# mmSir/SpatioTemporalEntropyModel

Hardware: AMD Instinct MI355X
Metric: frames/s (higher is better)
Workload: dtype f32; 1 GPU; configs[1]: SpatioTemporalPriorModel_Res(256,192) training step on mbt2018(192,192) latents, 16 septuplets x 7 frames x 256x256 per GPU, EMLoss, clip 1.0 + Adam 1e-4 / aux Adam 1e-3; per_gpu_batch=16, global_batch=16, parallelism=dp1, stream_priorities=latents=0,side=-1,compute=-1, stream_cu_masks=latents=block:160, plan_selectors=library defaults

## Files before the change

### __graft_entry__.py

```python
import os
import subprocess
import sys

REPO = os.path.dirname(os.path.abspath(__file__))
if REPO not in sys.path:
    sys.path.insert(0, REPO)


def build() -> None:
    env = dict(os.environ)
    jobs = str(min(8, os.cpu_count() or 1))
    subprocess.check_call(["make", "-C", os.path.join(REPO, "spatiotemporalentropymodel_amd", "csrc"), "-j", jobs], env=env)
    subprocess.check_call(["make", "-C", os.path.join(REPO, "oracle"), "all"], env=env)
    import spatiotemporalentropymodel_amd as pkg
    from spatiotemporalentropymodel_amd import _lib
    assert _lib.hip().stem_abi_version() == 5
    _lib.rans()
    _lib.frameio()
    _lib.roiio()


def smoke() -> None:
    from spatiotemporalentropymodel_amd.selfcheck import smoke_check
    smoke_check(verbose=True)


if __name__ == "__main__":
    build()
    if len(sys.argv) > 1 and sys.argv[1] == "smoke":
        smoke()
```

### spatiotemporalentropymodel_amd/_lib.py

```python
from __future__ import annotations

import ctypes as C
import os
import re

from . import _abi

_PKG = os.path.dirname(os.path.abspath(__file__))
HIP_SO = os.environ.get("STEM_HIP_LIBRARY") or os.path.join(_PKG, "libstem_hip.so")
RANS_SO = os.environ.get("STEM_RANS_LIBRARY") or os.path.join(_PKG, "libstem_rans.so")

FRAMEIO_SO = os.path.join(_PKG, "libstem_frameio.so")
ROIIO_SO = os.path.join(_PKG, "libstem_roiio.so")
DP_SO = os.environ.get("STEM_DP_LIBRARY") or os.path.join(_PKG, "libstem_dp.so")
_hip = None
_rans = None
_dp = None
_frameio = None
_roiio = None


class StemLibraryError(RuntimeError):
    pass


def _header(name):
    path = os.path.join(_PKG, "..", "include", name)
    if not os.path.exists(path):
        raise StemLibraryError(f"{path} is missing: the ctypes prototypes and structures are read from the C headers")
    return path


def _tables(header):
    protos = _abi.prototypes(_header(header))
    return protos, {n: args for n, (_, args) in protos.items()}, {n: res for n, (res, _) in protos.items() if res is not C.c_int}


_HIP_PROTO, _HIP_SIG, _RESTYPE = _tables("stem_hip.h")
_HIP_BATCH_PROTO, _HIP_BATCH_SIG, _ = _tables("stem_ar_batch.h")
_HIP_BLOCKS_PROTO, _HIP_BLOCKS_SIG, _ = _tables("stem_blocks.h")
_HIP_HYPERPRIOR_PROTO, _HIP_HYPERPRIOR_SIG, _ = _tables("stem_hyperprior.h")
_HIP_EBF_PROTO, _HIP_EBF_SIG, _ = _tables("stem_eb_filters.h")
_HIP_GDN1_PROTO, _HIP_GDN1_SIG, _ = _tables("stem_gdn1.h")
_HIP_VALIDATION_PROTO, _HIP_VALIDATION_SIG, _ = _tables("stem_validation.h")
_FRAMEIO_PROTO, _FRAMEIO_SIG, _ = _tables("stem_frameio.h")
_ROIIO_PROTO, _ROIIO_SIG, _ = _tables("stem_roiio.h")
_RANS_PROTO, _RANS_SIG, _RANS_RESTYPE = _tables("stem_rans.h")
_DP_PROTO, _DP_SIG, _ = _tables("stem_dp.h")
_STRUCTS = _abi.structs(_header("stem_hip.h"))


class PackDesc(C.Structure):
    _fields_ = _STRUCTS["stem_pack_desc"]


class F16PackDesc(C.Structure):
    _fields_ = _STRUCTS["stem_f16x2_pack_desc"]


class F16PairDesc(C.Structure):
    _fields_ = _STRUCTS["stem_f16x2_pair_desc"]


class UnpackDesc(C.Structure):
    _fields_ = _STRUCTS["stem_unpack_desc"]


class BiasFinalDesc(C.Structure):
    _fields_ = _STRUCTS["stem_bias_final_desc"]


class WaveSeg(C.Structure):
    _fields_ = _STRUCTS["stem_wave_seg"]


def _bind(lib, protos):
    for name, (restype, argtypes) in protos.items():
        fn = getattr(lib, name)
        fn.argtypes = argtypes
        fn.restype = restype
    return lib


def hip():
    global _hip
    if _hip is None:
        if not os.path.exists(HIP_SO):
            raise StemLibraryError(
                f"{HIP_SO} is missing: build it with `python -c 'import __graft_entry__ as g; g.build()'` "
                "(hipcc --offload-arch=gfx950).  There is no CPU fallback for the STEM kernels.")
        lib = C.CDLL(HIP_SO)
        for protos in (_HIP_PROTO, _HIP_BATCH_PROTO, _HIP_BLOCKS_PROTO, _HIP_HYPERPRIOR_PROTO, _HIP_EBF_PROTO, _HIP_GDN1_PROTO,
                       _HIP_VALIDATION_PROTO):
            _bind(lib, protos)
        _hip = lib
    return _hip


def frameio():
    global _frameio
    if _frameio is None:
        if not os.path.exists(FRAMEIO_SO):
            raise StemLibraryError(f"{FRAMEIO_SO} is missing: build it with `python -c 'import __graft_entry__ as g; g.build()'` "
                                   "(hipcc --offload-arch=gfx950).  There is no CPU fallback for the frame kernels.")
        _frameio = _bind(C.CDLL(FRAMEIO_SO), _FRAMEIO_PROTO)
    return _frameio


def check_frameio(rc: int):
    if rc != 0:
        raise RuntimeError((frameio().stem_frameio_last_error() or b"").decode() or f"libstem_frameio error {rc}")


def roiio():
    global _roiio
    if _roiio is None:
        if not os.path.exists(ROIIO_SO):
            raise StemLibraryError(f"{ROIIO_SO} is missing: build it with `python -c 'import __graft_entry__ as g; g.build()'` "
                                   "(hipcc --offload-arch=gfx950).  There is no CPU fallback for the frame kernels.")
        _roiio = _bind(C.CDLL(ROIIO_SO), _ROIIO_PROTO)
    return _roiio


def check_roiio(rc: int):
    if rc != 0:
        raise RuntimeError((roiio().stem_roiio_last_error() or b"").decode() or f"libstem_roiio error {rc}")


def rans():
    global _rans
    if _rans is None:
        if not os.path.exists(RANS_SO):
            raise StemLibraryError(f"{RANS_SO} is missing: run `make -C {os.path.join(_PKG, 'csrc')}`")
        _rans = _bind(C.CDLL(RANS_SO), _RANS_PROTO)
    return _rans


def check(rc: int):
    if rc != 0:
        raise RuntimeError((hip().stem_last_error() or b"").decode() or f"libstem_hip error {rc}")


def declared_hip_symbols():
    return sorted(_HIP_SIG)


def declared_hip_batch_symbols():
    return sorted(_HIP_BATCH_SIG)


def declared_hip_block_symbols():
    return sorted(_HIP_BLOCKS_SIG)


def declared_hip_hyperprior_symbols():
    return sorted(_HIP_HYPERPRIOR_SIG)


def declared_hip_eb_filters_symbols():
    return sorted(_HIP_EBF_SIG)


def declared_hip_gdn1_symbols():
    return sorted(_HIP_GDN1_SIG)


def declared_hip_validation_symbols():
    return sorted(_HIP_VALIDATION_SIG)


def declared_frameio_symbols():
    return sorted(_FRAMEIO_SIG)


def declared_roiio_symbols():
    return sorted(_ROIIO_SIG)


def header_macro(header, name):
    m = re.search(rf"^[ \t]*#[ \t]*define[ \t]+{name}[ \t]+(\d+)\b", open(_header(header)).read(), flags=re.M)
    if not m:
        raise StemLibraryError(f"include/{header} does not define {name} as an integer")
    return int(m.group(1))


def dp():
    global _dp
    if _dp is None:
        if not os.path.exists(DP_SO):
            raise StemLibraryError(f"{DP_SO} is missing: run `make -C {os.path.join(_PKG, 'csrc')}`")
        _dp = _bind(C.CDLL(DP_SO), _DP_PROTO)
    return _dp


def declared_dp_symbols():
    return sorted(_DP_SIG)


def declared_rans_symbols():
    return sorted(_RANS_SIG)
```

### spatiotemporalentropymodel_amd/config.py

```python
from __future__ import annotations

import contextlib
import dataclasses
import os
from dataclasses import dataclass


@dataclass
class StemRuntimeConfig:
    analysis_f16x3: bool = True
    first_layer_f16x3: bool = True
    engine_f16x3: bool = True
    engine_strided_f16x3: bool = True
    engine_transposed_f16x3: bool = True
    engine_ctx_f16x3: bool = True
    engine_wgrad_f16x3: bool = True
    engine_records: bool = True
    layers_f16x3: bool = True
    layers_f16x3_maxpix: int = 1 << 30
    layers_wide_minpix: int = 32768
    trainer_overwrite_grads: bool = True
    adam_block_max: bool = True
    engine_overlap: bool = True
    engine_split_pack: bool = True
    engine_pack_pair: bool = True
    engine_branch: bool = True
    stream_prio: str = ""
    stream_cumask: str = ""
    dp_threaded: int = 3
    dp_min_bytes: int = 8 << 20
    dist_backend: str = ""
    dist_single: bool = False
    pin_ranks: bool = True
    ar_persistent: bool = True
    ar_stepwise: bool = False
    ar_force_batch: bool = False
    ar_concurrent: bool = True
    ar_no_batch: bool = False


_ENV = {
    "analysis_f16x3": "STEM_F16X3", "first_layer_f16x3": "STEM_C4GDN_F16X3", "engine_f16x3": "STEM_ENGINE_F16X3",
    "engine_strided_f16x3": "STEM_ENGINE_STRIDED_F16X3", "engine_transposed_f16x3": "STEM_ENGINE_TRANSPOSED_F16X3", "engine_ctx_f16x3": "STEM_ENGINE_CTX_F16X3",
    "engine_wgrad_f16x3": "STEM_ENGINE_WGRAD_F16X3", "engine_records": "STEM_ENGINE_RECORDS", "layers_f16x3": "STEM_LAYERS_F16X3",
    "layers_f16x3_maxpix": "STEM_LAYERS_F16X3_MAXPIX", "layers_wide_minpix": "STEM_LAYERS_WIDE_MINPIX",
    "adam_block_max": "STEM_ADAM_BLOCK_MAX", "trainer_overwrite_grads": "STEM_TRAINER_OVERWRITE_GRADS", "engine_overlap": "STEM_ENGINE_OVERLAP",
    "engine_split_pack": "STEM_ENGINE_SPLIT_PACK", "engine_pack_pair": "STEM_ENGINE_PACK_PAIR", "engine_branch": "STEM_ENGINE_BRANCH",
    "stream_prio": "STEM_STREAM_PRIO", "stream_cumask": "STEM_STREAM_CUMASK", "dp_min_bytes": "STEM_DP_MIN_BYTES", "dp_threaded": "STEM_DP_THREADED",
    "dist_backend": "STEM_DIST_BACKEND", "dist_single": "STEM_DIST_SINGLE", "pin_ranks": "STEM_PIN_RANKS",
    "ar_persistent": "STEM_AR_PERSISTENT", "ar_stepwise": "STEM_AR_STEPWISE",
    "ar_force_batch": "STEM_AR_FORCE_BATCH", "ar_concurrent": "STEM_AR_CONCURRENT", "ar_no_batch": "STEM_AR_NO_BATCH",
}


def _parse(kind, text):
    if kind is bool:
        return text.strip() not in ("", "0", "false", "False", "no", "off")
    if kind is int:
        return int(text)
    return text


def from_env(environ=None) -> StemRuntimeConfig:
    environ = os.environ if environ is None else environ
    cfg = StemRuntimeConfig()
    for f in dataclasses.fields(cfg):
        name = _ENV[f.name]
        if name in environ:
            setattr(cfg, f.name, _parse(type(f.default), environ[name]))
    return cfg


_RUNTIME = None
_SNAPSHOT = None
_OVERRIDES = {}


def _snapshot():
    env = os.environ
    return tuple(env.get(v) for v in _ENV.values())


def runtime() -> StemRuntimeConfig:
    global _RUNTIME, _SNAPSHOT
    snap = _snapshot()
    if _RUNTIME is None or snap != _SNAPSHOT:
        _RUNTIME, _SNAPSHOT = from_env(), snap
        for k, v in _OVERRIDES.items():
            setattr(_RUNTIME, k, v)
    return _RUNTIME


def reload() -> StemRuntimeConfig:
    global _RUNTIME
    _RUNTIME = None
    return runtime()


@contextlib.contextmanager
def override(**fields):
    cfg = runtime()
    unknown = [k for k in fields if not hasattr(cfg, k)]
    if unknown:
        raise AttributeError(f"StemRuntimeConfig has no field(s) {unknown}")
    old = {k: (_OVERRIDES[k] if k in _OVERRIDES else None, k in _OVERRIDES, getattr(cfg, k)) for k in fields}
    try:
        for k, v in fields.items():
            _OVERRIDES[k] = v
            setattr(runtime(), k, v)
        yield runtime()
    finally:
        for k, (ov, had, val) in old.items():
            if had:
                _OVERRIDES[k] = ov
            else:
                _OVERRIDES.pop(k, None)
            setattr(runtime(), k, ov if had else val)
```

### spatiotemporalentropymodel_amd/csrc/optim.hip

```cpp
#include "stem_common.h"

namespace {

__global__ __launch_bounds__(256) void sumsq_kernel(const f32x4 *g4, const float *g, size_t n4, size_t n, double *part)
{
    __shared__ double red[256];
    double s = 0.0;
    for (size_t i = (size_t)blockIdx.x * 256 + threadIdx.x; i < n4; i += (size_t)gridDim.x * 256) {
        const f32x4 v = g4[i];
        s += (double)v[0] * v[0] + (double)v[1] * v[1] + (double)v[2] * v[2] + (double)v[3] * v[3];
    }
    if (blockIdx.x == 0)
        for (size_t i = n4 * 4 + threadIdx.x; i < n; i += 256) s += (double)g[i] * g[i];
    red[threadIdx.x] = s;
    __syncthreads();
    for (int k = 128; k > 0; k >>= 1) {
        if (threadIdx.x < k) red[threadIdx.x] += red[threadIdx.x + k];
        __syncthreads();
    }
    if (threadIdx.x == 0) part[blockIdx.x] = red[0];
}
__global__ __launch_bounds__(256) void sumsq_final_kernel(const double *part, int nparts, double *acc, int overwrite)
{
    __shared__ double red[256];
    double s = 0.0;
    for (int i = threadIdx.x; i < nparts; i += 256) s += part[i];
    red[threadIdx.x] = s;
    __syncthreads();
    for (int k = 128; k > 0; k >>= 1) {
        if (threadIdx.x < k) red[threadIdx.x] += red[threadIdx.x + k];
        __syncthreads();
    }
    if (threadIdx.x == 0) acc[0] = overwrite ? red[0] : acc[0] + red[0];
}

__global__ __launch_bounds__(256) void adam_kernel(float *p, float *g, float *m, float *v, size_t n, const double *sumsq,
                                                   float max_norm, float gscale, float step_size, float b1, float b2,
                                                   float inv_sqrt_bc2, float eps, const float *dev_scal, int zero_g)
{
    if (dev_scal) {
        step_size = dev_scal[0];
        inv_sqrt_bc2 = dev_scal[1];
    }
    float coef = gscale;
    if (max_norm > 0.f && sumsq) {
        const float total = (float)sqrt(sumsq[0]) * gscale;
        coef *= fminf(max_norm / (total + 1e-6f), 1.0f);
    }
    for (size_t i = (size_t)blockIdx.x * 256 + threadIdx.x; i < n; i += (size_t)gridDim.x * 256) {
        const float gi = g[i] * coef;
        if (zero_g) g[i] = 0.f;
        const float mi = m[i] + (gi - m[i]) * (1.f - b1);
        const float vi = v[i] * b2 + (1.f - b2) * gi * gi;
        m[i] = mi;
        v[i] = vi;
        p[i] -= step_size * (mi / (sqrtf(vi) * inv_sqrt_bc2 + eps));
    }
}

__global__ __launch_bounds__(256) void adam_bmax_kernel(float *p, float *g, float *m, float *v, size_t n, const double *sumsq,
                                                        float max_norm, float gscale, float step_size, float b1, float b2,
                                                        float inv_sqrt_bc2, float eps, int zero_g, float *bmax)
{
    float coef = gscale;
    if (max_norm > 0.f && sumsq) {
        const float total = (float)sqrt(sumsq[0]) * gscale;
        coef *= fminf(max_norm / (total + 1e-6f), 1.0f);
    }
    const size_t base = (size_t)blockIdx.x * STEM_ADAM_CHUNK;
    float mx = 0.f;
#pragma unroll 1
    for (int k0 = 0; k0 < STEM_ADAM_CHUNK / 256; k0 += 4) {
        float gi[4], mi[4], vi[4], pi[4];
        size_t idx[4];
#pragma unroll
        for (int u = 0; u < 4; ++u) {
            idx[u] = base + (size_t)(k0 + u) * 256 + threadIdx.x;
            const bool ok = idx[u] < n;
            const size_t j = ok ? idx[u] : 0;
            gi[u] = ok ? g[j] : 0.f;
            mi[u] = ok ? m[j] : 0.f;
            vi[u] = ok ? v[j] : 0.f;
            pi[u] = ok ? p[j] : 0.f;
        }
#pragma unroll
        for (int u = 0; u < 4; ++u) {
            if (idx[u] >= n) continue;
            const float gs = gi[u] * coef;
            if (zero_g) g[idx[u]] = 0.f;
            const float mn = mi[u] + (gs - mi[u]) * (1.f - b1);
            const float vn = vi[u] * b2 + (1.f - b2) * gs * gs;
            m[idx[u]] = mn;
            v[idx[u]] = vn;
            const float pn = pi[u] - step_size * (mn / (sqrtf(vn) * inv_sqrt_bc2 + eps));
            p[idx[u]] = pn;
            mx = fmaxf(mx, fabsf(pn));
        }
    }
    mx = wave_max(mx);
    if ((threadIdx.x & 63) == 0) bmax[blockIdx.x * 4 + (threadIdx.x >> 6)] = mx;
}

__global__ void adam_prepare_kernel(long long *step, const float *lr, float b1, float b2, float *scal)
{
    const long long t = step[0] + 1;
    step[0] = t;
    const double bc1 = 1.0 - pow((double)b1, (double)t), bc2 = 1.0 - pow((double)b2, (double)t);
    scal[0] = (float)((double)lr[0] / bc1);
    scal[1] = (float)(1.0 / sqrt(bc2));
}

__global__ void counter_add_kernel(long long *ctr, long long inc) { ctr[0] += inc; }

__global__ __launch_bounds__(256) void clip_scale_kernel(float *g, size_t n, const double *sumsq, float max_norm)
{
    const float coef = fminf(max_norm / ((float)sqrt(sumsq[0]) + 1e-6f), 1.0f);
    if (coef >= 1.0f) return;
    for (size_t i = (size_t)blockIdx.x * 256 + threadIdx.x; i < n; i += (size_t)gridDim.x * 256) g[i] *= coef;
}

__global__ __launch_bounds__(256) void axpy_kernel(float *y, const float *x, float a, size_t n)
{
    for (size_t i = (size_t)blockIdx.x * 256 + threadIdx.x; i < n; i += (size_t)gridDim.x * 256) y[i] += a * x[i];
}

}

namespace {
int sumsq_impl(const float *g, size_t n, double *acc, int overwrite, void *stream);
}
STEM_EXPORT int stem_sumsq(const float *g, size_t n, double *acc, void *stream) { return sumsq_impl(g, n, acc, 0, stream); }
STEM_EXPORT int stem_sumsq_set(const float *g, size_t n, double *acc, void *stream) { return sumsq_impl(g, n, acc, 1, stream); }
namespace {
int sumsq_impl(const float *g, size_t n, double *acc, int overwrite, void *stream)
{
    STEM_CHECK_ARG(g && acc, "stem_sumsq: null pointer");
    if (n == 0) {
        if (overwrite && hipMemsetAsync(acc, 0, sizeof(double), (hipStream_t)stream) != hipSuccess) return -2;
        return 0;
    }
    const bool al = (((uintptr_t)g) & 15) == 0;
    const size_t n4 = al ? n / 4 : 0;
    size_t nb = cdivz(n4 ? n4 : 1, 256);
    if (nb > STEM_SUMSQ_SCRATCH) nb = STEM_SUMSQ_SCRATCH;
    hipLaunchKernelGGL(sumsq_kernel, dim3((unsigned)nb), dim3(256), 0, (hipStream_t)stream,
                       reinterpret_cast<const f32x4 *>(g), g, n4, n, acc + 1);
    hipLaunchKernelGGL(sumsq_final_kernel, dim3(1), dim3(256), 0, (hipStream_t)stream, acc + 1, (int)nb, acc, overwrite);
    STEM_LAUNCH_CHECK("sumsq");
    return 0;
}
}

STEM_EXPORT int stem_adam_step(float *p, const float *g, float *m, float *v, size_t n, const double *sumsq, float max_norm,
                               float gscale, float lr, float beta1, float beta2, float eps, int step, void *stream)
{
    STEM_CHECK_ARG(p && g && m && v && step >= 1, "stem_adam_step: bad arguments");
    if (n == 0) return 0;
    const double bc1 = 1.0 - pow((double)beta1, step), bc2 = 1.0 - pow((double)beta2, step);
    size_t nb = cdivz(n, 256);
    if (nb > 4096) nb = 4096;
    hipLaunchKernelGGL(adam_kernel, dim3((unsigned)nb), dim3(256), 0, (hipStream_t)stream, p, const_cast<float *>(g), m, v, n, sumsq, max_norm,
                       gscale, (float)(lr / bc1), beta1, beta2, (float)(1.0 / sqrt(bc2)), eps, (const float *)nullptr, 0);
    STEM_LAUNCH_CHECK("adam");
    return 0;
}

STEM_EXPORT int stem_adam_step_zero(float *p, float *g, float *m, float *v, size_t n, const double *sumsq, float max_norm,
                                    float gscale, float lr, float beta1, float beta2, float eps, int step, void *stream)
{
    STEM_CHECK_ARG(p && g && m && v && step >= 1, "stem_adam_step_zero: bad arguments");
    if (n == 0) return 0;
    const double bc1 = 1.0 - pow((double)beta1, step), bc2 = 1.0 - pow((double)beta2, step);
    size_t nb = cdivz(n, 256);
    if (nb > 4096) nb = 4096;
    hipLaunchKernelGGL(adam_kernel, dim3((unsigned)nb), dim3(256), 0, (hipStream_t)stream, p, g, m, v, n, sumsq, max_norm,
                       gscale, (float)(lr / bc1), beta1, beta2, (float)(1.0 / sqrt(bc2)), eps, (const float *)nullptr, 1);
    STEM_LAUNCH_CHECK("adam_zero");
    return 0;
}

STEM_EXPORT size_t stem_adam_chunk(void) { return STEM_ADAM_CHUNK; }

STEM_EXPORT int stem_adam_step_bmax(float *p, float *g, float *m, float *v, size_t n, const double *sumsq, float max_norm,
                                    float gscale, float lr, float beta1, float beta2, float eps, int step, int zero_grad, float *bmax,
                                    void *stream)
{
    STEM_CHECK_ARG(p && g && m && v && bmax && step >= 1, "stem_adam_step_bmax: bad arguments");
    if (n == 0) return 0;
    const double bc1 = 1.0 - pow((double)beta1, step), bc2 = 1.0 - pow((double)beta2, step);
    hipLaunchKernelGGL(adam_bmax_kernel, dim3((unsigned)cdivz(n, STEM_ADAM_CHUNK)), dim3(256), 0, (hipStream_t)stream, p, g, m, v, n, sumsq,
                       max_norm, gscale, (float)(lr / bc1), beta1, beta2, (float)(1.0 / sqrt(bc2)), eps, zero_grad, bmax);
    STEM_LAUNCH_CHECK("adam_bmax");
    return 0;
}

STEM_EXPORT int stem_adam_step_dev(float *p, const float *g, float *m, float *v, size_t n, const double *sumsq, float max_norm,
                                   float gscale, const float *lr_dev, float beta1, float beta2, float eps, long long *step_dev,
                                   float *scal_dev, void *stream)
{
    STEM_CHECK_ARG(p && g && m && v && lr_dev && step_dev && scal_dev, "stem_adam_step_dev: null pointer");
    if (n == 0) return 0;
    hipLaunchKernelGGL(adam_prepare_kernel, dim3(1), dim3(1), 0, (hipStream_t)stream, step_dev, lr_dev, beta1, beta2, scal_dev);
    size_t nb = cdivz(n, 256);
    if (nb > 4096) nb = 4096;
    hipLaunchKernelGGL(adam_kernel, dim3((unsigned)nb), dim3(256), 0, (hipStream_t)stream, p, const_cast<float *>(g), m, v, n, sumsq, max_norm,
                       gscale, 0.f, beta1, beta2, 0.f, eps, (const float *)scal_dev, 0);
    STEM_LAUNCH_CHECK("adam_dev");
    return 0;
}

STEM_EXPORT int stem_counter_add(long long *ctr, long long inc, void *stream)
{
    STEM_CHECK_ARG(ctr, "stem_counter_add: null pointer");
    hipLaunchKernelGGL(counter_add_kernel, dim3(1), dim3(1), 0, (hipStream_t)stream, ctr, inc);
    STEM_LAUNCH_CHECK("counter_add");
    return 0;
}

STEM_EXPORT int stem_clip_scale(float *g, size_t n, const double *sumsq, float max_norm, void *stream)
{
    STEM_CHECK_ARG(g && sumsq && max_norm > 0.f, "stem_clip_scale: bad arguments");
    if (n == 0) return 0;
    size_t nb = cdivz(n, 256);
    if (nb > 4096) nb = 4096;
    hipLaunchKernelGGL(clip_scale_kernel, dim3((unsigned)nb), dim3(256), 0, (hipStream_t)stream, g, n, sumsq, max_norm);
    STEM_LAUNCH_CHECK("clip_scale");
    return 0;
}

STEM_EXPORT int stem_axpy(float *y, const float *x, float a, size_t n, void *stream)
{
    STEM_CHECK_ARG(y && x, "stem_axpy: null pointer");
    if (n == 0) return 0;
    size_t nb = cdivz(n, 256);
    if (nb > 4096) nb = 4096;
    hipLaunchKernelGGL(axpy_kernel, dim3((unsigned)nb), dim3(256), 0, (hipStream_t)stream, y, x, a, n);
    STEM_LAUNCH_CHECK("axpy");
    return 0;
}
```

### spatiotemporalentropymodel_amd/csrc/tape.hip

```cpp
#include <algorithm>
#include <array>
#include <type_traits>
#include <utility>
#include <vector>

#include "stem_common.h"

namespace {

constexpr int TAPE_MAXI = 40, TAPE_MAXF = 6;
enum { TAPE_CALL = 0, TAPE_WAIT = 1, TAPE_EVENT_RECORD = 2, TAPE_EVENT_WAIT = 3 };

struct TapeEntry {
    int kind;
    void *fn;
    int ni, nf;
    long long iv[TAPE_MAXI];
    long long idelta[TAPE_MAXI];
    double fv[TAPE_MAXF];
    hipStream_t s0, s1;
    hipEvent_t ev;
    bool dynamic;
};

struct Tape {
    std::vector<TapeEntry> e;
    std::vector<hipEvent_t> owned;
};

template <size_t... I, size_t... Fx>
int call_seq(void *fn, const long long *iv, const double *fv, std::index_sequence<I...>, std::index_sequence<Fx...>)
{
    using Fn = int (*)(decltype((void)I, 0LL)..., decltype((void)Fx, 0.0)...);
    return reinterpret_cast<Fn>(fn)(iv[I]..., fv[Fx]...);
}
template <size_t NI>
int call_ni(void *fn, const long long *iv, int nf, const double *fv)
{
    switch (nf) {
    case 0: return call_seq(fn, iv, fv, std::make_index_sequence<NI>{}, std::make_index_sequence<0>{});
    case 1: return call_seq(fn, iv, fv, std::make_index_sequence<NI>{}, std::make_index_sequence<1>{});
    case 2: return call_seq(fn, iv, fv, std::make_index_sequence<NI>{}, std::make_index_sequence<2>{});
    case 3: return call_seq(fn, iv, fv, std::make_index_sequence<NI>{}, std::make_index_sequence<3>{});
    case 4: return call_seq(fn, iv, fv, std::make_index_sequence<NI>{}, std::make_index_sequence<4>{});
    case 5: return call_seq(fn, iv, fv, std::make_index_sequence<NI>{}, std::make_index_sequence<5>{});
    default: return call_seq(fn, iv, fv, std::make_index_sequence<NI>{}, std::make_index_sequence<6>{});
    }
}
using Caller = int (*)(void *, const long long *, int, const double *);
template <size_t... N>
constexpr auto make_callers(std::index_sequence<N...>) -> std::array<Caller, sizeof...(N)>
{
    return {{&call_ni<N>...}};
}
const auto kCallers = make_callers(std::make_index_sequence<TAPE_MAXI + 1>{});

static_assert(TAPE_MAXF <= 8, "SSE arguments beyond xmm7 go to the stack and would interleave with the integer overflow area");
template <class T>
constexpr bool tape_int_class = (std::is_integral<T>::value || std::is_enum<T>::value || std::is_pointer<T>::value) && sizeof(T) <= 8;
template <class T>
constexpr bool tape_sse_class = std::is_same<T, float>::value || std::is_same<T, double>::value;
template <class... A>
constexpr bool tape_recordable(int (*)(A...))
{
    constexpr int ni = (0 + ... + (tape_int_class<A> ? 1 : 0)), nf = (0 + ... + (tape_sse_class<A> ? 1 : 0));
    return ni + nf == (int)sizeof...(A) && ni <= TAPE_MAXI && nf <= TAPE_MAXF;
}
#define STEM_TAPE_ENTRY(name) \
    static_assert(tape_recordable(&name), #name ": prototype outside the launch tape's calling contract (csrc/tape.hip)");
#include "tape_entries.inc"
#undef STEM_TAPE_ENTRY

#define STEM_TAPE_ENTRY(name) reinterpret_cast<const void *>(&name),
const void *const kRecordable[] = {
#include "tape_entries.inc"
};
#undef STEM_TAPE_ENTRY

}

STEM_EXPORT int stem_tape_entry_recordable(void *fn)
{
    return std::find(std::begin(kRecordable), std::end(kRecordable), (const void *)fn) != std::end(kRecordable) ? 1 : 0;
}

STEM_EXPORT void *stem_tape_create(void) { return new Tape(); }

STEM_EXPORT void stem_tape_destroy(void *tape)
{
    Tape *t = static_cast<Tape *>(tape);
    if (!t) return;
    for (hipEvent_t ev : t->owned) (void)hipEventDestroy(ev);
    delete t;
}

STEM_EXPORT int stem_tape_length(void *tape) { return tape ? (int)static_cast<Tape *>(tape)->e.size() : -1; }

STEM_EXPORT int stem_tape_add_call(void *tape, void *fn, int nargs, const unsigned char *kinds, const long long *ivals, const double *fvals,
                                   const long long *ideltas)
{
    Tape *t = static_cast<Tape *>(tape);
    STEM_CHECK_ARG(t && fn && nargs >= 0 && (nargs == 0 || (kinds && ivals && fvals)), "stem_tape_add_call: null argument");
    TapeEntry en;
    memset(&en, 0, sizeof(en));
    en.kind = TAPE_CALL;
    en.fn = fn;
    for (int i = 0; i < nargs; ++i) {
        if (kinds[i] != 0) {
            STEM_CHECK_ARG(en.nf < TAPE_MAXF, "stem_tape_add_call: more than %d float arguments", TAPE_MAXF);
            en.fv[en.nf++] = fvals[i];
        } else {
            STEM_CHECK_ARG(en.ni < TAPE_MAXI, "stem_tape_add_call: more than %d integer-class arguments", TAPE_MAXI);
            en.iv[en.ni] = ivals[i];
            en.idelta[en.ni] = ideltas ? ideltas[i] : 0;
            en.dynamic = en.dynamic || en.idelta[en.ni] != 0;
            ++en.ni;
        }
    }
    t->e.push_back(en);
    return (int)t->e.size() - 1;
}

STEM_EXPORT int stem_tape_add_wait(void *tape, void *waiting, void *signalling)
{
    Tape *t = static_cast<Tape *>(tape);
    STEM_CHECK_ARG(t, "stem_tape_add_wait: null tape");
    TapeEntry en;
    memset(&en, 0, sizeof(en));
    en.kind = TAPE_WAIT;
    en.s0 = (hipStream_t)waiting;
    en.s1 = (hipStream_t)signalling;
    if (hipEventCreateWithFlags(&en.ev, hipEventDisableTiming) != hipSuccess) {
        stem_set_error("stem_tape_add_wait: hipEventCreate failed");
        return -2;
    }
    t->owned.push_back(en.ev);
    t->e.push_back(en);
    return (int)t->e.size() - 1;
}

STEM_EXPORT int stem_tape_add_event(void *tape, void *event, void *stream, int wait)
{
    Tape *t = static_cast<Tape *>(tape);
    STEM_CHECK_ARG(t && event, "stem_tape_add_event: null argument");
    TapeEntry en;
    memset(&en, 0, sizeof(en));
    en.kind = wait ? TAPE_EVENT_WAIT : TAPE_EVENT_RECORD;
    en.s0 = (hipStream_t)stream;
    en.ev = (hipEvent_t)event;
    t->e.push_back(en);
    return (int)t->e.size() - 1;
}

STEM_EXPORT int stem_tape_replay(void *tape, int lo, int hi, long long n)
{
    Tape *t = static_cast<Tape *>(tape);
    STEM_CHECK_ARG(t && lo >= 0 && hi <= (int)t->e.size() && lo <= hi, "stem_tape_replay: bad range [%d, %d)", lo, hi);
    for (int i = lo; i < hi; ++i) {
        const TapeEntry &en = t->e[i];
        switch (en.kind) {
        case TAPE_CALL: {
            int rc;
            if (en.dynamic) {
                long long iv[TAPE_MAXI];
                for (int k = 0; k < en.ni; ++k) iv[k] = en.iv[k] + n * en.idelta[k];
                rc = kCallers[en.ni](en.fn, iv, en.nf, en.fv);
            } else {
                rc = kCallers[en.ni](en.fn, en.iv, en.nf, en.fv);
            }
            if (rc != 0) return -(i + 1);
            break;
        }
        case TAPE_WAIT:
            if (hipEventRecord(en.ev, en.s1) != hipSuccess || hipStreamWaitEvent(en.s0, en.ev, 0) != hipSuccess) {
                stem_set_error("stem_tape_replay: stream hand-over of entry %d failed", i);
                return -(i + 1);
            }
            break;
        case TAPE_EVENT_RECORD:
            if (hipEventRecord(en.ev, en.s0) != hipSuccess) {
                stem_set_error("stem_tape_replay: event record of entry %d failed", i);
                return -(i + 1);
            }
            break;
        default:
            if (hipStreamWaitEvent(en.s0, en.ev, 0) != hipSuccess) {
                stem_set_error("stem_tape_replay: event wait of entry %d failed", i);
                return -(i + 1);
            }
        }
    }
    return 0;
}

STEM_EXPORT int stem_tape_set_iarg(void *tape, int entry, int arg, long long value)
{
    Tape *t = static_cast<Tape *>(tape);
    STEM_CHECK_ARG(t && entry >= 0 && entry < (int)t->e.size() && t->e[entry].kind == TAPE_CALL && arg >= 0 && arg < t->e[entry].ni,
                   "stem_tape_set_iarg: no integer argument %d in entry %d", arg, entry);
    t->e[entry].iv[arg] = value;
    return 0;
}

STEM_EXPORT int stem_tape_set_farg(void *tape, int entry, int arg, double pattern)
{
    Tape *t = static_cast<Tape *>(tape);
    STEM_CHECK_ARG(t && entry >= 0 && entry < (int)t->e.size() && t->e[entry].kind == TAPE_CALL && arg >= 0 && arg < t->e[entry].nf,
                   "stem_tape_set_farg: no float argument %d in entry %d", arg, entry);
    t->e[entry].fv[arg] = pattern;
    return 0;
}

STEM_EXPORT int stem_zero_bytes(void *dst, size_t nbytes, void *stream)
{
    STEM_CHECK_ARG(dst || !nbytes, "stem_zero_bytes: null pointer");
    if (nbytes && hipMemsetAsync(dst, 0, nbytes, (hipStream_t)stream) != hipSuccess) {
        stem_set_error("stem_zero_bytes: hipMemsetAsync failed");
        return -2;
    }
    return 0;
}

STEM_EXPORT int stem_stream_flag_create(void **flag)
{
    STEM_CHECK_ARG(flag, "stem_stream_flag_create: null pointer");
    int dev = 0, ok = 0;
    if (hipGetDevice(&dev) != hipSuccess || hipDeviceGetAttribute(&ok, hipDeviceAttributeCanUseStreamWaitValue, dev) != hipSuccess || !ok) {
        stem_set_error("stem_stream_flag_create: this device / runtime has no stream wait-value operation");
        return -3;
    }
    void *p = nullptr;
    if (hipExtMallocWithFlags(&p, 8, hipMallocSignalMemory) != hipSuccess || !p) {
        stem_set_error("stem_stream_flag_create: hipExtMallocWithFlags(hipMallocSignalMemory) failed");
        return -2;
    }
    *static_cast<volatile uint64_t *>(p) = 0;
    *flag = p;
    return 0;
}

STEM_EXPORT int stem_stream_flag_destroy(void *flag)
{
    if (flag && hipFree(flag) != hipSuccess) {
        stem_set_error("stem_stream_flag_destroy: hipFree failed");
        return -2;
    }
    return 0;
}

STEM_EXPORT int stem_stream_flag_wait_ge(void *flag, unsigned value, void *stream)
{
    STEM_CHECK_ARG(flag, "stem_stream_flag_wait_ge: null flag");
    if (hipStreamWaitValue32((hipStream_t)stream, flag, value, hipStreamWaitValueGte, 0xffffffffu) != hipSuccess) {
        stem_set_error("stem_stream_flag_wait_ge: hipStreamWaitValue32 failed");
        return -2;
    }
    return 0;
}

STEM_EXPORT int stem_stream_flag_write(void *flag, unsigned value, void *stream)
{
    STEM_CHECK_ARG(flag, "stem_stream_flag_write: null flag");
    if (stream == (void *)-1) {
        __atomic_store_n(static_cast<uint32_t *>(flag), value, __ATOMIC_RELEASE);
        return 0;
    }
    if (hipStreamWriteValue32((hipStream_t)stream, flag, value, 0) != hipSuccess) {
        stem_set_error("stem_stream_flag_write: hipStreamWriteValue32 failed");
        return -2;
    }
    return 0;
}

STEM_EXPORT int stem_copy_d2d(void *dst, const void *src, size_t nbytes, void *stream)
{
    STEM_CHECK_ARG(dst && src, "stem_copy_d2d: null pointer");
    if (nbytes && hipMemcpyAsync(dst, src, nbytes, hipMemcpyDeviceToDevice, (hipStream_t)stream) != hipSuccess) {
        stem_set_error("stem_copy_d2d: hipMemcpyAsync failed");
        return -2;
    }
    return 0;
}
```

### spatiotemporalentropymodel_amd/engine.py

```python
from __future__ import annotations

import collections

import torch

from . import _lib
from . import config as _config
from . import functional as F
from . import layers as _layers

class _Switch:

    def __init__(self, field):
        self.field = field

    def __get__(self, obj, owner=None):
        return getattr(_config._RUNTIME or _config.runtime(), self.field)


class _Act:
    __slots__ = ("x", "p", "rec")

    def __init__(self, x, p=None, rec=None):
        self.x, self.p, self.rec = x, p, rec

    def planes(self, record=True):
        if self.p is None:
            self.p = F.F16Planes.split(self.x, src_q=self.rec.data_ptr() if record and self.rec is not None else None)
        return self.p

    def channels(self, c0, c1):
        return _Act(self.x[:, c0:c1], None if self.p is None else self.p.channels(c0, c1))


_Face = collections.namedtuple("_Face", "kind N C flip taps")


class _Layer:

    def __init__(self, mod, kind, eng):
        self.mod, self.kind, self.eng = mod, kind, eng
        self.R = mod.kernel_size
        self.stride, self.pad = mod.stride, mod.padding
        self.opad = getattr(mod, "output_padding", 0)
        self.K, self.C = mod.out_channels, mod.in_channels
        self.masked = getattr(mod, "_masked", 0)
        self.wp_fwd = self.wp_dgrad = None
        self.need_dgrad = True
        self.fx3 = False
        self.wg3 = False
        self.taps = 0
        self.fx3s = False
        self.fx3t = False
        self.wp6_fwd = self.wp6_dgrad = None
        self._slabs = {}
        self.pending = None
        self.lane = 0

    def fx3_eligible(self):
        return self.kind == "conv" and not self.masked and _layers.f16x3_same_shape(self.stride, self.R, self.pad, self.C, self.K)

    def fx3_masked_eligible(self):
        return (self.kind == "conv" and bool(self.masked) and not self.need_dgrad
                and _layers.f16x3_same_shape(self.stride, self.R, self.pad, self.C, self.K, k_multiple=4))

    def fx3s_eligible(self):
        n_out, n_red = (self.K, self.C) if self.kind == "conv" else (self.C, self.K)
        return (self.stride == 2 and not self.masked and n_red % 32 == 0 and n_out % 4 == 0 and self.R * self.R <= 25
                and (self.kind == "conv" or self.need_dgrad))

    def fx3t_eligible(self):
        return (self.fx3s and self.R % 2 == 1 and self.R >= 3 and self.pad == self.R // 2 and self.C % 32 == 0 and self.K % 32 == 0
                and (self.kind == "conv" or self.opad == 1))

    def wg3_eligible(self):
        return self.kind == "conv" and _layers.f16x3_same_shape(self.stride, self.R, self.pad, self.C, self.K)

    def set_faces(self):
        K, C, conv = self.K, self.C, self.kind == "conv"
        fwd = dgrad = _Face("f32", K, C, 0, 0)
        if self.fx3:
            fwd, dgrad = _Face("gen", K, C, 0, self.taps), _Face("gen", C, K, 1, 0)
        elif self.fx3s:
            if conv:
                fwd, dgrad = _Face("gen", K, C, 0, 0), (_Face("phases", C, K, 2, 0) if self.fx3t else dgrad)
            else:
                fwd, dgrad = (_Face("phases", K, C, 2, 0) if self.fx3t else fwd), _Face("gen", C, K, 0, 0)
        self.faces = (fwd, dgrad if self.need_dgrad else None)

    def alloc_packs(self, device):
        bufs = []
        for face in self.faces:
            if face is None:
                bufs += [None, None]
            elif face.kind == "f32":
                bufs += [torch.empty(self.K * self.C * self.R * self.R, device=device, dtype=torch.float32), None]
            else:
                bufs += [None, torch.zeros(F.f16x2_gen_weight_bytes(face.N, face.C, self.R, self.R), device=device, dtype=torch.uint8)]
        self.wp_fwd, self.wp6_fwd, self.wp_dgrad, self.wp6_dgrad = bufs
        if self.fx3s and self.wp_fwd is None:
            self.wp_fwd = torch.empty(0, device=device)

    def role_descs(self, role):
        face = self.faces[role]
        if face is None:
            return [], []
        if face.kind == "f32":
            return [self._desc32(role)], []
        wp = self.wp6_dgrad if role else self.wp6_fwd
        return [], [_lib.F16PackDesc(self.mod.weight.data_ptr(), wp.data_ptr(), face.N, face.C, self.R, self.R, face.flip, face.taps)]

    def pair_desc(self):
        a, b = self.role_descs(0), self.role_descs(1)
        if a[0] or b[0] or not a[1]:
            return None
        w = self.mod.weight
        A, Bd = int(w.shape[0]), int(w.shape[1])
        roles = []
        for d in (a[1][0], b[1][0] if b[1] else None):
            if d is None:
                roles += [None, 0, 0]
                continue
            rows_b = int(d.flip != 0)
            assert (d.N, d.C) == ((Bd, A) if rows_b else (A, Bd)), "pair pack: a role image must be a transpose of the tensor itself"
            roles += [d.wp, rows_b | (int(d.flip) << 1), int(d.taps)]
        return _lib.F16PairDesc(w.data_ptr(), A, Bd, self.R, self.R, roles[0], roles[1], roles[2], roles[3], roles[4], roles[5], None, 0, 0)

    def _desc32(self, role):
        w = self.mod.weight
        conv = self.kind == "conv"
        if role == 0:
            return _lib.PackDesc(w.data_ptr(), self.wp_fwd.data_ptr(), self.K, self.C, self.R, self.R,
                                 F.PACK_CONV_FWD if conv else F.PACK_DECONV_FWD, self.masked)
        return _lib.PackDesc(w.data_ptr(), self.wp_dgrad.data_ptr(), self.K, self.C, self.R, self.R,
                             F.PACK_CONV_DGRAD if conv else F.PACK_DECONV_DGRAD, (1 | (self.masked & 4)) if self.masked else 0)

    def forward(self, a, act=F.ACT_NONE, out=None, planes=False):
        self.eng.ensure_packed()
        face, m = self.faces[0], self.mod
        epi = F.GEN_EPI_LRELU if act == F.ACT_LRELU else F.GEN_EPI_BIAS
        if face.kind == "gen":
            return _Act(*F.conv2d_f16x3_gen(a.planes(), self.wp6_fwd, m.bias, self.K, self.R, self.R, self.stride, self.pad,
                                            epi=epi, out=out, want_planes=planes, taps=self.taps))
        if face.kind == "phases":
            return _Act(*F.tconv2d_f16x3(a.planes(), self.wp6_fwd, m.bias, self.K, self.R, epi=epi, out=out, want_planes=planes))
        self.eng._wait_fwd32_packs()
        if self.kind == "conv":
            if self.masked and not self.masked & 4:
                act |= F.CONV_MASKED_A
            return _Act(F.conv2d_fwd(a.x, self.wp_fwd, m.bias, self.K, self.R, self.R, self.stride, self.pad, act, out=out))
        return _Act(F.deconv2d_fwd(a.x, self.wp_fwd, m.bias, self.K, self.R, self.R, self.stride, self.pad, self.opad, act, out=out))

    def fwd(self, x, act=F.ACT_NONE, out=None):
        return self.forward(_Act(x), act, out=out).x

    def input_grad(self, dy, xact=None, planes=False, x_shape=None):
        face = self.faces[1]
        epi = F.GEN_EPI_DACT if xact is not None else F.GEN_EPI_BIAS
        if face.kind == "gen":
            return _Act(*F.conv2d_f16x3_gen(dy.planes(), self.wp6_dgrad, None, self.C, self.R, self.R, self.stride, self.pad,
                                            epi=epi, z=xact, want_planes=planes))
        if face.kind == "phases":
            return _Act(*F.tconv2d_f16x3(dy.planes(), self.wp6_dgrad, None, self.C, self.R, epi=epi, z=xact, want_planes=planes,
                                         fine_hw=tuple(xact.shape[2:]) if xact is not None else None))
        x_shape = xact.shape if xact is not None else x_shape
        if self.kind == "conv":
            return _Act(F.conv2d_dgrad(dy.x, self.wp_dgrad, x_shape, self.K, self.R, self.R, self.stride, self.pad, xact=xact))
        return _Act(F.deconv2d_dgrad(dy.x, self.wp_dgrad, x_shape, self.K, self.R, self.R, self.stride, self.pad, self.opad, xact=xact))

    def reads_dy_planes(self, x):
        return self.faces[1].kind != "f32" if self.faces[1] is not None else (self.wg3 and x.p is not None)

    def weight_grad(self, x, dy):
        at_hand = (x.p is not None) + (dy.p is not None)
        if self.fx3t:
            fn, args = self._wgrad_t, ((x.planes(), dy.planes()) if self.kind == "conv" else (dy.planes(), x.planes())) + (dy.x,)
        elif self.wg3 and at_hand >= (2 if self.need_dgrad else 1):
            fn, args = self._wgrad3, (x.planes(record=False), dy.planes(record=False), dy.x)
        else:
            fn, args = self._wgrad, (x.x, dy.x)
        side = self.eng.side_stream(dy.x.device, self.lane)
        if side is None:
            return fn(*args)
        F.stream_wait(side, F.cur_stream(dy.x.device))
        with F.on_stream(side):
            fn(*args)
        for t in args:
            (t.data if isinstance(t, F.F16Planes) else t).record_stream(side)

    def _wgrad_t(self, fine_p, coarse_p, dy):
        conv = self.kind == "conv"
        Kk = self.K if conv else self.C
        key = ("fp16t",) + tuple(fine_p.shape)
        if key not in self._slabs:
            splits, elems = F.wgrad_f16x3_strided_plan(fine_p.shape, Kk, self.R, self.R, self.stride, self.pad)
            self._slabs[key] = (torch.empty(elems, device=dy.device, dtype=torch.float32), splits,
                                torch.empty(splits * Kk, device=dy.device, dtype=torch.float32))
        dwp, splits, bpart = self._slabs[key]
        gb = _grad_of(self.mod.bias) if self.mod.bias is not None else None
        F.conv2d_wgrad_f16x3_strided(fine_p, coarse_p, Kk, self.R, self.R, self.stride, self.pad, dwp, splits,
                                     bias_part=bpart if (conv and gb is not None) else None)
        self.pending_bias = None
        if gb is not None and conv:
            self.pending_bias = _lib.BiasFinalDesc(bpart.data_ptr(), gb.data_ptr(), self.K, splits, int(self.eng.accumulate_grads), 0)
        elif gb is not None:
            F.bias_grad(dy, gb, accumulate=self.eng.accumulate_grads)
        self.pending = (dwp, splits)

    def _wgrad3(self, xp, dyp, dy):
        key = ("fp16",) + tuple(xp.shape)
        if key not in self._slabs:
            splits, elems = F.wgrad_f16x3_plan(xp.shape, self.K, self.R, self.R, self.pad)
            self._slabs[key] = (torch.empty(elems, device=dy.device, dtype=torch.float32), splits,
                                torch.empty(splits * self.K, device=dy.device, dtype=torch.float32))
        dwp, splits, bpart = self._slabs[key]
        gb = _grad_of(self.mod.bias) if self.mod.bias is not None else None
        self.pending_bias = F.conv2d_wgrad_f16x3(xp, dyp, self.K, self.R, self.R, self.pad, dwp, splits, db=gb, bias_part=bpart,
                                                 accumulate_db=self.eng.accumulate_grads, defer_bias=True)
        self.pending = (dwp, splits)

    def _wgrad(self, x, dy):
        m = self.mod
        gb = _grad_of(m.bias)
        deconv = self.kind == "deconv"
        key = tuple(x.shape)
        key = key + (F.nhwc_ld(x), F.nhwc_ld(dy))
        fresh = key not in self._slabs
        if fresh:
            splits, elems = F.wgrad_plan(x.shape, self.K, self.R, self.R, self.stride, self.pad, deconv=deconv)
            self._slabs[key] = (torch.empty(elems, device=x.device, dtype=torch.float32), splits)
        dwp, splits = self._slabs[key]
        defer = gb is not None
        if deconv:
            _, b = F.deconv2d_wgrad(x, dy, self.K, self.R, self.R, self.stride, self.pad, self.opad, db_out=gb, dwp=dwp, unpack=False,
                                    table_valid=not fresh, accumulate_db=self.eng.accumulate_grads, defer_bias=defer)
        else:
            _, b = F.conv2d_wgrad(x, dy, self.K, self.R, self.R, self.stride, self.pad, db_out=gb, dwp=dwp, unpack=False,
                                  table_valid=not fresh, accumulate_db=self.eng.accumulate_grads, defer_bias=defer)
        self.pending_bias = b if defer else None
        self.pending = (dwp, splits)

    def unpack_desc(self):
        dwp, splits = self.pending
        self.pending = None
        return _lib.UnpackDesc(dwp.data_ptr(), _grad_of(self.mod.weight).data_ptr(), self.K, self.C, self.R, self.R, splits,
                               (F.UNPACK_DECONV if self.kind == "deconv" else 0) | (F.UNPACK_ACCUMULATE if self.eng.accumulate_grads else 0))


def _attach_block_maxima(d, numel, maxima, flat, ch=None):
    off = (d.w - flat.data_ptr()) // 4
    if (d.w - flat.data_ptr()) % 4 or off < 0 or off + numel > flat.numel():
        return False
    ch = ch or F.adam_chunk()
    d.bmax, d.b0 = maxima.data_ptr(), off // ch
    d.nb = (off + numel - 1) // ch - d.b0 + 1
    return True


def _grad_of(p):
    if p.grad is None:
        owner = getattr(p, "_flat_grad_view", None)
        p.grad = owner if owner is not None else torch.zeros_like(p, memory_format=torch.contiguous_format)
    return p.grad


class StemEngine:
    def __init__(self, model, has_tpm: bool, has_spm: bool, residual: bool):
        _config.runtime()
        self.m = model
        eb_filters = tuple(model.entropy_bottleneck.filters)
        if eb_filters != (3, 3, 3, 3):
            raise ValueError(f"StemEngine: the fused schedule is built for an EntropyBottleneck with filters=(3, 3, 3, 3), this model's "
                             f"has filters={eb_filters}; its module-by-module forward (model(y_cur, y_conditioned)) and autograd work")
        self.has_tpm, self.has_spm, self.residual = has_tpm, has_spm, residual
        L = lambda mod: _Layer(mod, "conv", self)
        D = lambda mod: _Layer(mod, "deconv", self)
        self.HE = [L(model.HE[0]), L(model.HE[2]), L(model.HE[4])]
        self.HD = [D(model.HD[0]), D(model.HD[2]), L(model.HD[4])]
        self.TPM = [L(model.TPM[0]), L(model.TPM[2]), L(model.TPM[4])] if has_tpm else None
        self.CTX = L(model.context_prediction) if has_spm else None
        self.EPM = [L(model.EPM[0]), L(model.EPM[2]), L(model.EPM[4])]
        self.nprior = 1 + int(has_tpm) + int(has_spm)
        self.layers = self.HE + self.HD + (self.TPM or []) + ([self.CTX] if has_spm else []) + self.EPM
        for first in [self.HE[0]] + ([self.TPM[0]] if has_tpm else []) + ([self.CTX] if has_spm else []):
            first.need_dgrad = False
        self._pack_key = None
        self._side = {}
        self._checked = False
        self._dgrad_pack_event = None
        self._fwd32_pack_event = None
        self.accumulate_grads = True
        self._events = {}
        self._select_fx3()

    def _select_fx3(self):
        for l in self.layers:
            l.fx3 = self.use_fx3 and l.fx3_eligible()
            l.taps = 0
            l.fx3s = False
        if self.use_fx3 and self.use_fx3s:
            if self.HE[0].fx3 and self.HE[1].fx3s_eligible():
                self.HE[1].fx3s = True
                self.HE[2].fx3s = self.HE[2].fx3s_eligible() and self.HE[1].K % 32 == 0
            if self.HD[2].fx3 and self.HD[1].fx3s_eligible():
                self.HD[1].fx3s = True
                self.HD[0].fx3s = self.HD[0].fx3s_eligible() and self.HD[1].C % 32 == 0
        if self.use_fx3t and self.use_wg3:
            for l in self.HE[1:] + self.HD[:2]:
                l.fx3t = l.fx3t_eligible()
            if not (self.HE[1].fx3t and self.HE[2].fx3t and self.HE[0].fx3):
                self.HE[1].fx3t = self.HE[2].fx3t = False
            if not (self.HD[0].fx3t and self.HD[1].fx3t and self.HD[2].fx3):
                self.HD[0].fx3t = self.HD[1].fx3t = False
        if self.has_spm and self.use_fx3 and self.use_ctx3 and self.CTX.fx3_masked_eligible():
            self.CTX.fx3 = True
            self.CTX.taps = F.masked_live_taps(self.CTX.R, self.CTX.R, "B" if self.CTX.masked & 4 else "A")
        P = self.HE[0].C
        for group, need_aligned in ((self.TPM, False), (self.EPM, True)):
            if group and not (all(l.fx3 for l in group) and (not need_aligned or P % 32 == 0)):
                for l in group:
                    l.fx3 = False
        for l in self.layers:
            l.wg3 = self.use_fx3 and self.use_wg3 and l.wg3_eligible()
            l.set_faces()

    use_fx3 = _Switch("engine_f16x3")
    use_records = _Switch("engine_records")
    use_fx3s = _Switch("engine_strided_f16x3")
    use_fx3t = _Switch("engine_transposed_f16x3")
    use_ctx3 = _Switch("engine_ctx_f16x3")
    use_wg3 = _Switch("engine_wgrad_f16x3")

    overlap_wgrad = _Switch("engine_overlap")

    split_pack = _Switch("engine_split_pack")

    def side_stream(self, device, lane=0):
        if not self.overlap_wgrad or device.type != "cuda" or lane < 0:
            return None
        st = self._side.get(lane)
        if st is None or st.device != device:
            st = self._side[lane] = F.make_stream(device, "side")
        return st

    branch_streams = _Switch("engine_branch")

    def _branch(self, device, which=0):
        if not self.branch_streams or device.type != "cuda":
            return None
        bs = getattr(self, "_bstreams", None)
        if bs is None:
            bs = self._bstreams = {}
        st = bs.get(which)
        if st is None or st.device != device:
            st = bs[which] = F.make_stream(device, "branch")
        return st

    def ensure_packed(self, block_max=None, split=True):
        if self._checked:
            return
        if self._weights_key() == self._pack_key:
            return
        have = [l.wp_fwd if l.faces[0].kind == "f32" else l.wp6_fwd for l in self.layers]
        if any(h is None or h.device != l.mod.weight.device for h, l in zip(have, self.layers)):
            for l in self.layers:
                l.alloc_packs(l.mod.weight.device)
        dev = self.layers[0].mod.weight.device
        if block_max is not None and self.pack_pair and self._pack_pairs(*block_max):
            self._pack_key = self._weights_key()
            return
        side = self.side_stream(dev) if split and self.split_pack and not torch.cuda.is_current_stream_capturing() else None
        if not split:
            for st in list(self._side.values()) + list(getattr(self, "_bstreams", {}).values()):
                F.stream_wait(F.cur_stream(dev), st)
            self._dgrad_pack_event = None
        roles = ((0, 1), (1, 2)) if side is not None else ((0, 2),)
        for lo, hi in roles:
            on_side = side is not None and lo == 1
            if on_side:
                F.stream_wait(side, F.cur_stream(dev))
            with F.on_stream(side if on_side else None):
                both = [l.role_descs(r) for l in self.layers for r in range(lo, hi)]
                descs = [d for a, _ in both for d in a]
                descs6 = [d for _, b in both for d in b]
                if descs6 and block_max is not None:
                    ch = F.adam_chunk()
                    for d in descs6:
                        _attach_block_maxima(d, d.N * d.C * d.R * d.S, *block_max, ch)
                if descs6:
                    F.pack_weights_f16x2_multi((_lib.F16PackDesc * len(descs6))(*descs6))
                bs = self._branch(dev) if (descs and side is not None and not on_side and lo == 0 and hi == 1) else None
                if descs and bs is not None:
                    F.stream_wait(bs, F.cur_stream(dev))
                    with F.on_stream(bs):
                        F.pack_weights_multi((_lib.PackDesc * len(descs))(*descs))
                        self._fwd32_pack_event = self._events.setdefault("fwd32", torch.cuda.Event())
                        F.event_record(self._fwd32_pack_event, bs)
                elif descs:
                    F.pack_weights_multi((_lib.PackDesc * len(descs))(*descs))
                    if not on_side:
                        self._fwd32_pack_event = None
                if on_side:
                    self._dgrad_pack_event = self._events.setdefault("dgrad", torch.cuda.Event())
                    F.event_record(self._dgrad_pack_event, side)
        self._pack_key = self._weights_key()

    def _weights_key(self):
        return tuple((_layers.weight_epoch(l.mod.weight), l.mod.weight._version, l.mod.weight.data_ptr()) for l in self.layers)

    pack_pair = _Switch("engine_pack_pair")

    def _pack_pairs(self, maxima, flat):
        descs = [l.pair_desc() for l in self.layers]
        if any(d is None for d in descs):
            return False
        ch = F.adam_chunk()
        if not all(_attach_block_maxima(d, d.A * d.B * d.R * d.S, maxima, flat, ch) for d in descs):
            return False
        F.pack_weights_f16x2_pair_multi((_lib.F16PairDesc * len(descs))(*descs))
        self._dgrad_pack_event = None
        return True

    def unpack_all(self):
        for lane in sorted({l.lane for l in self.layers}):
            self._group_ready([l for l in self.layers if l.lane == lane], [])

    grad_ready_hook = None

    def _group_ready(self, layers, extra_params):
        dev = layers[0].mod.weight.device
        side = self.side_stream(dev, layers[0].lane)
        if side is None:
            return self._group_ready_on_stream(layers, extra_params)
        F.stream_wait(side, F.cur_stream(dev))
        with F.on_stream(side):
            self._group_ready_on_stream(layers, extra_params)

    def _group_ready_on_stream(self, layers, extra_params):
        bdescs = [l.pending_bias for l in layers if getattr(l, "pending_bias", None) is not None]
        for l in layers:
            l.pending_bias = None
        if bdescs:
            F.bias_grad_final_multi(bdescs)
        descs = [l.unpack_desc() for l in layers if l.pending is not None]
        if descs:
            arr = (_lib.UnpackDesc * len(descs))(*descs)
            F.unpack_wgrads_multi(arr)
        if self.grad_ready_hook is not None:
            params = [p for l in layers for p in (l.mod.weight, l.mod.bias) if p is not None] + list(extra_params)
            if params:
                hook = self.grad_ready_hook
                F.tape_py(lambda: hook(params))

    def join_side_stream(self):
        for st in self._side.values():
            F.stream_wait(F.cur_stream(st.device), st)

    def _wait_fwd32_packs(self):
        if self._fwd32_pack_event is not None:
            F.event_wait(F.cur_stream(), self._fwd32_pack_event)

    def _wait_dgrad_packs(self):
        if self._dgrad_pack_event is not None:
            F.event_wait(F.cur_stream(), self._dgrad_pack_event)
            self._dgrad_pack_event = None

    def forward(self, y_cur, y_cond, training: bool, rate_coef=None):
        self.ensure_packed()
        self._checked = True
        try:
            return self._forward(y_cur, y_cond, training, rate_coef)
        finally:
            self._checked = False

    @staticmethod
    def _chain_forward(layers, a, out=None, planes=True):
        acts = [a]
        for i, l in enumerate(layers):
            nxt = layers[i + 1] if i + 1 < len(layers) else None
            acts.append(l.forward(acts[-1], F.ACT_LRELU if nxt else F.ACT_NONE, out=None if nxt else out,
                                  planes=planes and nxt is not None and nxt.faces[0].kind != "f32"))
        return acts

    @staticmethod
    def _chain_backward(layers, xs, dy, planes=False):
        for i in range(len(layers) - 1, -1, -1):
            l = layers[i]
            if l.faces[1] is not None and l.faces[1].kind != "f32":
                dy.planes()
            l.weight_grad(xs[i], dy)
            if l.faces[1] is None:
                return None
            dy = l.input_grad(dy, xact=xs[i].x if i else None, x_shape=xs[i].x.shape,
                              planes=layers[i - 1].reads_dy_planes(xs[i - 1]) if i else planes)
        return dy

    def _forward(self, y_cur, y_cond, training: bool, rate_coef=None):
        m = self.m
        yc, yd = F.to_nhwc(y_cur.detach()), F.to_nhwc(y_cond.detach())
        B, Cin, H, W = yc.shape
        dev = yc.device
        eb, gc = m.entropy_bottleneck, m.gaussian_conditional
        fused = rate_coef is not None
        assert not fused or training, "the fused glue is the TRAINING forward"
        k = {}
        target = t_hat = y_hat = None
        ep = training or self.has_spm
        rec = {}
        if fused:
            slot = gc._noise_slot(yc) if self.has_spm else {}
            he_in, target, t_hat, y_hat = F.prior_prologue(yc, yd, self.residual, True, self.has_spm, records=rec if self.use_fx3 and self.use_records else None, **slot)
        else:
            he_in = F.empty_nhwc(B, 2 * Cin, H, W, dev)
            F.copy_channels(yc, he_in[:, :Cin])
            F.copy_channels(yd, he_in[:, Cin:])
        P = 2 * Cin
        epm_in = F.empty_nhwc(B, self.nprior * P, H, W, dev)
        o_tp, o_hp = (0, P) if self.has_tpm else (None, 0)
        o_ctx = o_hp + P
        bs = self._branch(dev)
        main = F.cur_stream(dev) if bs is not None else None
        if bs is not None:
            F.stream_wait(bs, main)
        acts = k["acts"] = {}
        acts["he_in"] = _Act(he_in, rec=rec.get("in"))
        acts["yd"] = _Act(yd, rec=rec.get("in"))
        ctx_split_done = None
        if self.has_spm and fused:
            acts["t_hat"] = _Act(t_hat, rec=rec.get("t_hat"))
            if self.CTX.fx3 and rec.get("t_hat") is not None and self.side_stream(dev) is not None:
                side = self.side_stream(dev)
                F.stream_wait(side, F.cur_stream(dev))
                with F.on_stream(side):
                    acts["t_hat"].planes()
                    ctx_split_done = self._events.setdefault("ctx_split", torch.cuda.Event())
                    F.event_record(ctx_split_done, side)
                t_hat.record_stream(side)

        if fused and self.HE[0].fx3 and self.has_tpm and self.TPM[0].fx3 and Cin % 32 == 0 and rec.get("in") is not None:
            acts["yd"] = _Act(yd, acts["he_in"].planes().channels(Cin, 2 * Cin))
            if bs is not None:
                F.stream_wait(bs, main)

        tp0 = tp2 = None
        if self.has_tpm:
            _, acts["tp0"], acts["tp2"], _ = self._chain_forward(self.TPM, acts["yd"], out=epm_in[:, o_tp:o_tp + P], planes=ep)
            tp0, tp2 = acts["tp0"].x, acts["tp2"].x
        with F.on_stream(bs):
            _, acts["he0"], acts["he2"], z = self._chain_forward(self.HE, acts["he_in"], planes=ep)
            z = z.x
            pack = F.eb_pack(eb._tensors14())
            if fused:
                if self.HD[0].fx3t and self.use_records:
                    z_hat, lik_z, k["dlik_z"], part_z, rec["z_hat"] = F.eb_forward_train(z, pack, rate_coef[0], bound=eb._lik_bound, record=True,
                                                                                         **eb._noise_slot(z))
                else:
                    z_hat, lik_z, k["dlik_z"], part_z = F.eb_forward_train(z, pack, rate_coef[0], bound=eb._lik_bound, **eb._noise_slot(z))
            elif training:
                z_hat, lik_z = F.eb_forward(z, pack, noise=eb._noise_like(z))
            else:
                z_hat, lik_z = F.eb_forward(z, pack, medians=eb._medians_vec())
            acts["z_hat"], acts["hd0"], acts["hd2"], _ = self._chain_forward(self.HD, _Act(z_hat, rec=rec.get("z_hat")), out=epm_in[:, o_hp:o_hp + P], planes=ep)
        if not fused:
            target = F.sub(yc, yd) if self.residual else (yc if F.nhwc_ld(yc) == Cin else F.copy_channels(yc, F.empty_nhwc(B, Cin, H, W, dev)))
        if self.has_spm:
            if not fused:
                t_hat = F.add(target, gc._noise_like(target)) if training else F.round_(target)
                acts["t_hat"] = _Act(t_hat)
            if ctx_split_done is not None:
                F.event_wait(F.cur_stream(dev), ctx_split_done)
            self.CTX.forward(acts["t_hat"], out=epm_in[:, o_ctx:o_ctx + P])
        if bs is not None:
            F.stream_wait(main, bs)
        acts["epm_in"], acts["e0"], acts["e2"], gp = self._chain_forward(self.EPM, _Act(epm_in), planes=ep)
        gp = gp.x
        scales, means = gp[:, :Cin], gp[:, Cin:]
        if fused:
            dgp = F.empty_nhwc(B, 2 * Cin, H, W, dev)
            gc_out, lik_y, k["dlik_y"], part_y, k["qg"] = F.gc_forward_train(
                target, scales, means, rate_coef[0], scale_bound=gc._scale_bound, lik_bound=gc._lik_bound,
                backward=(dgp[:, :Cin], dgp[:, Cin:]), record=self.EPM[0].fx3 and self.use_records, **gc._noise_slot(target))
            k["dgp"] = dgp
            k["loss3"] = F.em_loss_finalize(part_y, part_z, rate_coef[1])
            if not self.has_spm:
                y_hat = gc_out
        else:
            noise = gc._noise_like(target) if training else None
            gc_out, lik_y = F.gc_forward(target, scales, means, noise=noise, scale_bound=gc._scale_bound, lik_bound=gc._lik_bound)
            if self.has_spm:
                y_hat = F.add(t_hat, yd if F.nhwc_ld(yd) == Cin else F.copy_channels(yd, F.empty_nhwc(B, Cin, H, W, dev))) if self.residual else t_hat
            else:
                y_hat = gc_out
        k.update(he_in=he_in, he0=acts["he0"].x, he2=acts["he2"].x, z_hat=z_hat, pack=pack, hd0=acts["hd0"].x, hd2=acts["hd2"].x,
                 epm_in=epm_in, tp0=tp0, tp2=tp2, yd=yd, t_hat=t_hat, e0=acts["e0"].x, e2=acts["e2"].x, gp=gp, gc_out=gc_out,
                 offs=(o_tp, o_hp, o_ctx), P=P, Cin=Cin)
        return y_hat, lik_y, lik_z, k

    def eval_rate(self, y_cur, y_cond, num_pixels, acc=None, weight=1.0):
        self.ensure_packed()
        self._checked = True
        try:
            return self._eval_rate(y_cur, y_cond, num_pixels, acc, weight)
        finally:
            self._checked = False

    def _eval_rate(self, y_cur, y_cond, num_pixels, acc, weight):
        m = self.m
        yc, yd = F.to_nhwc(y_cur.detach()), F.to_nhwc(y_cond.detach())
        B, Cin, H, W = yc.shape
        dev = yc.device
        eb, gc = m.entropy_bottleneck, m.gaussian_conditional
        ep = self.has_spm
        he_in, target, t_hat, y_hat = F.prior_prologue(yc, yd, self.residual, False, self.has_spm, records=None)
        P = 2 * Cin
        epm_in = F.empty_nhwc(B, self.nprior * P, H, W, dev)
        o_tp, o_hp = (0, P) if self.has_tpm else (None, 0)
        o_ctx = o_hp + P
        bs = self._branch(dev)
        main = F.cur_stream(dev) if bs is not None else None
        if bs is not None:
            F.stream_wait(bs, main)
        if self.has_tpm:
            self._chain_forward(self.TPM, _Act(yd), out=epm_in[:, o_tp:o_tp + P], planes=ep)
        with F.on_stream(bs):
            z = self._chain_forward(self.HE, _Act(he_in), planes=ep)[-1].x
            z_hat, lik_z, part_z = F.eb_forward_eval_rate(z, F.eb_pack(eb._tensors14()), eb._medians_vec())
            self._chain_forward(self.HD, _Act(z_hat), out=epm_in[:, o_hp:o_hp + P], planes=ep)
        if self.has_spm:
            self.CTX.forward(_Act(t_hat), out=epm_in[:, o_ctx:o_ctx + P])
        if bs is not None:
            F.stream_wait(main, bs)
            for t in (lik_z, part_z):
                t.record_stream(main)
        gp = self._chain_forward(self.EPM, _Act(epm_in), planes=ep)[-1].x
        gc_out, lik_y, part_y = F.gc_forward_eval_rate(target, gp[:, :Cin], gp[:, Cin:], scale_bound=gc._scale_bound, lik_bound=gc._lik_bound)
        if acc is None:
            acc = torch.zeros(4, dtype=torch.float64, device=dev)
        loss3 = F.em_loss_accumulate(part_y, part_z, -1.0 / num_pixels, acc, weight=weight)
        return (y_hat if self.has_spm else gc_out), lik_y, lik_z, loss3

    def backward(self, k, dlik_y, dlik_z):
        m = self.m
        gc = m.gaussian_conditional
        Cin, P = k["Cin"], k["P"]
        o_tp, o_hp, o_ctx = k["offs"]
        gp, acts = k["gp"], k["acts"]
        B, _, H, W = gp.shape
        self._wait_dgrad_packs()
        if k.get("dgp") is not None and dlik_y is k.get("dlik_y"):
            dgp, qg = k["dgp"], k["qg"]
        else:
            dgp = F.empty_nhwc(B, 2 * Cin, H, W, gp.device)
            qg = F.gc_backward(k["gc_out"], gp[:, :Cin], gp[:, Cin:], dlik_y, dgp[:, :Cin], dgp[:, Cin:], dy=None,
                               scale_bound=gc._scale_bound, lik_bound=gc._lik_bound, record=self.EPM[0].fx3 and self.use_records)
        dpri = self._chain_backward(self.EPM, [acts["epm_in"], acts["e0"], acts["e2"]], _Act(dgp, rec=qg), planes=True)
        self._group_ready(self.EPM, [])
        bs = self._branch(gp.device)
        main = F.cur_stream(gp.device)

        if bs is not None:
            epm_done = self._events.setdefault("bwd_epm", torch.cuda.Event())
            F.event_record(epm_done, main)
        if self.has_spm:
            self._chain_backward([self.CTX], [acts["t_hat"]], dpri.channels(o_ctx, o_ctx + P))
            self._group_ready([self.CTX], [])
        if self.has_tpm:
            for l in self.TPM:
                l.lane = -1 if bs is not None else 0
            self._chain_backward(self.TPM, [acts["yd"], acts["tp0"], acts["tp2"]], dpri.channels(o_tp, o_tp + P))
            self._group_ready(self.TPM, [])
        if bs is None:
            self._backward_hyper(k, dpri.channels(o_hp, o_hp + P), dlik_z)
        else:
            F.event_wait(bs, epm_done)
            with F.on_stream(bs):
                self._backward_hyper(k, dpri.channels(o_hp, o_hp + P), dlik_z)
            F.stream_wait(main, bs)
        self.join_side_stream()

    def _backward_hyper(self, k, dhp, dlik_z):
        acts = k["acts"]
        dz_hat = self._chain_backward(self.HD, [acts["z_hat"], acts["hd0"], acts["hd2"]], dhp).x
        eb = self.m.entropy_bottleneck
        qdz = None
        if self.HE[2].fx3t and self.use_records:
            dz, dpack, qdz = F.eb_backward(k["z_hat"], k["pack"], dlik_z, dzhat_in=dz_hat, bound=eb._lik_bound, record=True)
        else:
            dz, dpack = F.eb_backward(k["z_hat"], k["pack"], dlik_z, dzhat_in=dz_hat, bound=eb._lik_bound)
        F.eb_unpack_grads(dpack, [_grad_of(p) for p in eb._tensors14()], accumulate=self.accumulate_grads)
        self._group_ready(self.HD, eb._tensors14())
        self._chain_backward(self.HE, [acts["he_in"], acts["he0"], acts["he2"]], _Act(dz, rec=qdz))
        self._group_ready(self.HE, [])


class StemFunction(torch.autograd.Function):

    @staticmethod
    def forward(ctx, engine, training, y_cur, y_cond, *params):
        y_hat, lik_y, lik_z, k = engine.forward(y_cur, y_cond, training)
        ctx.engine, ctx.keep = engine, k
        ctx.mark_non_differentiable(y_hat)
        return y_hat, lik_y, lik_z

    @staticmethod
    def backward(ctx, _dy_hat, dlik_y, dlik_z):
        eng, k = ctx.engine, ctx.keep
        if k is None:
            raise RuntimeError("StemFunction: backward through this forward a second time -- its saved activations were "
                               "released by the first backward (retain_graph is not supported by the fused schedule; "
                               "run the forward again)")
        ctx.keep = None
        gp = k["gp"]
        B, _, H, W = gp.shape
        if dlik_y is None:
            dlik_y = torch.zeros_like(k["gc_out"])
        if dlik_z is None:
            dlik_z = torch.zeros_like(k["z_hat"])
        eng.backward(k, _dense(dlik_y), _dense(dlik_z))
        return (None,) * (4 + len(eng.m._engine_params))


def _dense(t):
    t = F.to_nhwc(t)
    if F.nhwc_ld(t) != t.shape[1]:
# ... 3 lines not shown
```

### spatiotemporalentropymodel_amd/functional.py

```python
from __future__ import annotations

import ctypes as C
import functools
import os

import torch

from . import _lib
from . import config as _config

PACK_CONV_FWD, PACK_CONV_DGRAD, PACK_DECONV_FWD, PACK_DECONV_DGRAD, PACK_CONV_FWD_C4 = 0, 1, 2, 3, 4
ACT_NONE, ACT_LRELU = 0, 1
CONV_MASKED_A = 0x100
LRELU_SLOPE = 0.01
EB_NPARAM = 58


def _stream():
    try:
        return torch._C._cuda_getCurrentRawStream(torch._C._cuda_getDevice())
    except AttributeError:
        return torch.cuda.current_stream().cuda_stream


# ... 1346 lines not shown
    _require_cuda(x)
    if x.dim() != 3 or x.numel() == 0:
        raise ValueError(f"plane_resample2 takes planes [P,H,W], got {tuple(x.shape)}")
    P, H, W = x.shape
    if mode == 2 and (H % 2 or W % 2):
        raise ValueError(f"the 2 x 2 mean needs even sides, got {H} x {W}")
    x = x.detach().contiguous()
    out = torch.empty((P, H // 2, W // 2) if mode == 2 else (P, 2 * H, 2 * W), dtype=torch.float32, device=x.device)
    _chk(_lib.hip().stem_plane_resample2(x.data_ptr(), out.data_ptr(), P, H, W, int(mode), _stream()))
    return out


def weighted_sqerr_bwd(xhat, x, lam, g, coef):
    B, Cc, H, W = xhat.shape
    g = g.to(torch.float64).contiguous()
    out = torch.empty_like(xhat)
    _chk(_lib.hip().stem_weighted_sqerr_bwd(xhat.data_ptr(), x.data_ptr(), lam.data_ptr(), out.data_ptr(), B, Cc, H * W, g.data_ptr(),
                                            float(coef), _stream()))
    return out


EB_TENSORS = [f"_{k}{i}" for i in range(5) for k in (("matrix", "bias", "factor") if i < 4 else ("matrix", "bias"))]


def _ptr_array(tensors):
    arr = (C.c_void_p * len(tensors))(*[t.data_ptr() for t in tensors])
    return arr


def eb_pack(tensors14):
    Cc = tensors14[0].shape[0]
    ts = [t.detach().contiguous() for t in tensors14]
    pack = torch.empty((Cc, EB_NPARAM), device=ts[0].device, dtype=torch.float32)
    _chk(_lib.hip().stem_eb_pack(_ptr_array(ts), pack.data_ptr(), Cc, _stream()))
    return pack


def eb_unpack_grads(dpack, grads14, accumulate=False):
    Cc = dpack.shape[0]
    _chk(_lib.hip().stem_eb_unpack_grads(dpack.data_ptr(), _ptr_array(grads14), Cc, 1 if accumulate else 0, _stream()))


def eb_forward(z, pack, medians=None, noise=None, bound=1e-9):
    B, Cc, H, W = z.shape
    z_hat, lik = empty_nhwc(B, Cc, H, W, z.device), empty_nhwc(B, Cc, H, W, z.device)
    mode = 0 if noise is not None else 1
    if noise is not None:
        assert nhwc_ld(noise) == Cc
    _chk(_lib.hip().stem_eb_forward(z.data_ptr(), nhwc_ld(z), _ptr(noise), pack.data_ptr(), _ptr(medians), z_hat.data_ptr(),
                                    lik.data_ptr(), B, H, W, Cc, mode, bound, _stream()))
    return z_hat, lik


def eb_backward(z_hat, pack, dlik, dzhat_in=None, bound=1e-9, record=False):
    B, Cc, H, W = z_hat.shape
    dz = empty_nhwc(B, Cc, H, W, z_hat.device)
    dpack = torch.empty_like(pack)
    if record:
        q = torch.empty(16 + Cc, device=z_hat.device, dtype=torch.float32)
        _chk(_lib.hip().stem_eb_backward_rec(z_hat.data_ptr(), pack.data_ptr(), dlik.data_ptr(), _ptr(dzhat_in), dz.data_ptr(),
                                             dpack.data_ptr(), B, H, W, Cc, bound, q.data_ptr(), _stream()))
        return dz, dpack, q
    _chk(_lib.hip().stem_eb_backward(z_hat.data_ptr(), pack.data_ptr(), dlik.data_ptr(), _ptr(dzhat_in), dz.data_ptr(),
                                     dpack.data_ptr(), B, H, W, Cc, bound, _stream()))
    return dz, dpack


def eb_aux_loss(quantiles, pack, target, need_grad=True):
    Cc = quantiles.shape[0]
    loss = torch.empty(1, device=quantiles.device, dtype=torch.float32)
    dq = torch.empty_like(quantiles) if need_grad else None
    _chk(_lib.hip().stem_eb_aux_loss(quantiles.detach().contiguous().data_ptr(), pack.data_ptr(), target.data_ptr(),
                                     loss.data_ptr(), _ptr(dq), Cc, _stream()))
    return loss, dq


def gc_forward(y, scales, means, noise=None, scale_bound=0.11, lik_bound=1e-9):
    B, Cc, H, W = y.shape
    assert nhwc_ld(y) == Cc
    ldsm = nhwc_ld(scales)
    assert ldsm == nhwc_ld(means)
    out, lik = empty_nhwc(B, Cc, H, W, y.device), empty_nhwc(B, Cc, H, W, y.device)
    mode = 0 if noise is not None else 1
    _chk(_lib.hip().stem_gc_forward(y.data_ptr(), _ptr(noise), scales.data_ptr(), means.data_ptr(), ldsm, out.data_ptr(),
                                    lik.data_ptr(), B * H * W, Cc, mode, scale_bound, lik_bound, _stream()))
    return out, lik


def qrec_for(nelem, device):
    return torch.empty(16 + (nelem + 255) // 256, device=device, dtype=torch.float32)


def gc_backward(out, scales, means, dlik, dscales, dmeans, dy=None, scale_bound=0.11, lik_bound=1e-9, record=False):
    B, Cc, H, W = out.shape
    ldd = nhwc_ld(dscales)
    assert ldd == nhwc_ld(dmeans)
    q = qrec_for(B * H * W * Cc, out.device) if record else None
    _chk(_lib.hip().stem_gc_backward(out.data_ptr(), scales.data_ptr(), means.data_ptr(), nhwc_ld(scales), dlik.data_ptr(),
                                     dscales.data_ptr(), dmeans.data_ptr(), ldd, _ptr(dy), B * H * W, Cc, scale_bound,
                                     lik_bound, _ptr(q), _stream()))
    return q


def gc_scale_forward(y, scales, mode="round", noise=None, seed=0, offset=0, epoch=None, scale_bound=0.11, lik_bound=1e-9):
    if mode not in ("noise", "round"):
        raise ValueError(f'gc_scale_forward: mode is "noise" or "round", got {mode!r}')
    B, Cc, H, W = y.shape
    if tuple(scales.shape) != tuple(y.shape) or (noise is not None and tuple(noise.shape) != tuple(y.shape)):
        raise ValueError(f"gc_scale_forward: y {tuple(y.shape)}, scales {tuple(scales.shape)}"
                         + ("" if noise is None else f", noise {tuple(noise.shape)}") + " differ in shape")
    (yp, ldy), (sp, lds) = _nhwc_arg(y, "gc_scale_forward: y"), _nhwc_arg(scales, "gc_scale_forward: scales")
    np_, ldn = _nhwc_arg(noise, "gc_scale_forward: noise") if noise is not None and mode == "noise" else (None, 0)
    out, lik = empty_nhwc(B, Cc, H, W, y.device), empty_nhwc(B, Cc, H, W, y.device)
    _, sd, off, ep, stride = _noise_args(None, seed, offset, epoch)
    _chk(_lib.hip().stem_gc_scale_forward(yp, ldy, np_, ldn, sd, off, ep, stride, sp, lds, out.data_ptr(), Cc, lik.data_ptr(), Cc,
                                          B * H * W, Cc, 0 if mode == "noise" else 1, scale_bound, lik_bound, _stream()))
    return out, lik


def gc_scale_backward(out, scales, dlik, dscales=None, dy=None, dout=None, scale_bound=0.11, lik_bound=1e-9, record=False):
    B, Cc, H, W = out.shape
    if dout is not None and dy is None:
        raise ValueError("gc_scale_backward: dout is added into dy, which is missing")
    args = []
    for t, name in ((out, "out"), (scales, "scales"), (dlik, "dlik"), (dout, "dout"), (dscales, "dscales"), (dy, "dy")):
        if t is None:
            args += [None, 0]
            continue
        assert tuple(t.shape) == tuple(out.shape), name
        args += _nhwc_arg(t, f"gc_scale_backward: {name}")
    q = qrec_for(B * H * W * Cc, out.device) if record else None
    _chk(_lib.hip().stem_gc_scale_backward(*args, B * H * W, Cc, scale_bound, lik_bound, _ptr(q), _stream()))
    return q


def abs_(x):
    B, Cc, H, W = x.shape
    out = empty_nhwc(B, Cc, H, W, x.device)
    xp, ldx = _nhwc_arg(x, "abs_: x")
    _chk(_lib.hip().stem_abs_fwd(xp, ldx, out.data_ptr(), Cc, B * H * W, Cc, _stream()))
    return out


def abs_backward(x, g):
    B, Cc, H, W = x.shape
    assert tuple(g.shape) == tuple(x.shape)
    dx = empty_nhwc(B, Cc, H, W, x.device)
    (xp, ldx), (gp, ldg) = _nhwc_arg(x, "abs_backward: x"), _nhwc_arg(g, "abs_backward: g")
    _chk(_lib.hip().stem_abs_bwd(xp, ldx, gp, ldg, dx.data_ptr(), Cc, B * H * W, Cc, _stream()))
    return dx


def log2_sum(lik, acc):
    _chk(_lib.hip().stem_log2_sum(lik.data_ptr(), lik.numel(), acc.data_ptr(), _stream()))


def dlog(lik, coef):
    out = torch.empty_like(lik)
    _chk(_lib.hip().stem_dlog(lik.data_ptr(), out.data_ptr(), lik.numel(), coef, _stream()))
    return out


def _dense_like(a):
    B, Cc, H, W = a.shape
    return empty_nhwc(B, Cc, H, W, a.device)


def sub(a, b):
    assert nhwc_ld(a) == a.shape[1] and nhwc_ld(b) == b.shape[1]
    out = _dense_like(a)
    _chk(_lib.hip().stem_sub(a.data_ptr(), b.data_ptr(), out.data_ptr(), a.numel(), _stream()))
    return out


def add(a, b):
    assert nhwc_ld(a) == a.shape[1] and nhwc_ld(b) == b.shape[1]
    out = _dense_like(a)
    _chk(_lib.hip().stem_add(a.data_ptr(), b.data_ptr(), out.data_ptr(), a.numel(), _stream()))
    return out


def round_(a):
    assert nhwc_ld(a) == a.shape[1]
    out = _dense_like(a)
    _chk(_lib.hip().stem_round(a.data_ptr(), out.data_ptr(), a.numel(), _stream()))
    return out


NOISE_EPOCH_STRIDE = 1 << 40


def uniform_noise_like(a, seed: int, offset: int, epoch=None):
    out = _dense_like(a)
    if epoch is None:
        _chk(_lib.hip().stem_uniform_noise(out.data_ptr(), out.numel(), seed & (2 ** 64 - 1), offset & (2 ** 64 - 1), _stream()))
    else:
        assert epoch.dtype == torch.int64 and epoch.is_cuda
        _chk(_lib.hip().stem_uniform_noise_epoch(out.data_ptr(), out.numel(), seed & (2 ** 64 - 1), offset & (2 ** 64 - 1),
                                                 epoch.data_ptr(), NOISE_EPOCH_STRIDE, _stream()))
    return out


def counter_add_(ctr, inc=1):
    assert ctr.dtype == torch.int64 and ctr.is_cuda
    _chk(_lib.hip().stem_counter_add(ctr.data_ptr(), int(inc), _stream()))
    return ctr


def build_indexes(scales, table, scale_bound=0.11):
    B, Cc, H, W = scales.shape
    idx = torch.empty((B, H, W, Cc), device=scales.device, dtype=torch.int32).permute(0, 3, 1, 2)
    _chk(_lib.hip().stem_build_indexes(scales.data_ptr(), nhwc_ld(scales), table.data_ptr(), table.numel(), idx.data_ptr(),
                                       B * H * W, Cc, scale_bound, _stream()))
    return idx


def _pitch(t, name, shape):
    _require_cuda(t)
    ld = nhwc_ld(t)
    if tuple(t.shape) != tuple(shape) or ld is None:
        raise ValueError(f"{name}: expected an NHWC-memory tensor of shape {tuple(shape)}, got {tuple(t.shape)} with strides {t.stride()}")
    return ld


def _chan_vec(v, Cc, name):
    _require_cuda(v)
    if v.dim() != 1 or v.numel() != Cc or not v.is_contiguous():
        raise ValueError(f"{name}: expected a dense vector of {Cc} values, got {tuple(v.shape)}")
    return v


def symbols_pack(y=None, means=None, chan_means=None, scales=None, table=None, scale_bound=0.11, want_indexes=True, out=None):
    ref = y if y is not None else scales
    if ref is None:
        raise ValueError("symbols_pack: one of y / scales is needed (channel-number indexes alone need no device)")
    shape = tuple(ref.shape)
    B, Cc, H, W = (int(s) for s in shape)
    device = ref.device
    if scales is not None and table is None:
        raise ValueError("symbols_pack: scales need their table")
    si = out if out is not None else torch.empty((2, B, Cc, H, W), device=device, dtype=torch.int32)
    assert si.dtype == torch.int32 and si.is_contiguous() and tuple(si.shape) == (2, B, Cc, H, W)
    ldy = _pitch(y, "y", shape) if y is not None else 0
    ldm = _pitch(means, "means", shape) if means is not None else 0
    lds = _pitch(scales, "scales", shape) if scales is not None else 0
    if chan_means is not None:
        _chan_vec(chan_means, Cc, "chan_means")
    if table is not None:
        _require_cuda(table)
        assert table.is_contiguous()
    _chk(_lib.hip().stem_symbols_pack(_ptr(y), ldy, _ptr(means), ldm, _ptr(chan_means), _ptr(scales), lds,
                                      _ptr(table) if scales is not None else 0, table.numel() if scales is not None else 0,
                                      float(scale_bound), si[0].data_ptr() if y is not None else 0,
                                      si[1].data_ptr() if want_indexes else 0, B, H, W, Cc, _stream()))
    return si


def symbols_unpack(sym, means=None, chan_means=None, out=None):
    if not sym.is_cuda or sym.dtype != torch.int32 or sym.dim() != 4 or not sym.is_contiguous():
        raise RuntimeError("symbols_unpack expects a dense int32 [B,C,H,W] device tensor (no CPU fallback exists)")
    B, Cc, H, W = sym.shape
    ldm = _pitch(means, "means", sym.shape) if means is not None else 0
    if chan_means is not None:
        _chan_vec(chan_means, Cc, "chan_means")
    y_hat = out if out is not None else empty_nhwc(B, Cc, H, W, sym.device)
    ldo = _pitch(y_hat, "out", sym.shape)
    _chk(_lib.hip().stem_symbols_unpack(sym.data_ptr(), _ptr(means), ldm, _ptr(chan_means), y_hat.data_ptr(), ldo, B, H, W, Cc, _stream()))
    return y_hat


SUMSQ_SCRATCH = 2048


def sumsq_accumulator(device):
    return torch.zeros(1 + SUMSQ_SCRATCH, dtype=torch.float64, device=device)


def sumsq(g, acc, overwrite=False):
    assert acc.numel() >= 1 + SUMSQ_SCRATCH
    fn = _lib.hip().stem_sumsq_set if overwrite else _lib.hip().stem_sumsq
    _chk(fn(g.data_ptr(), g.numel(), acc.data_ptr(), _stream()))


def clip_scale(g, sumsq_acc, max_norm):
    _chk(_lib.hip().stem_clip_scale(g.data_ptr(), g.numel(), sumsq_acc.data_ptr(), float(max_norm), _stream()))


def axpy_(y, x, a):
    _chk(_lib.hip().stem_axpy(y.data_ptr(), x.data_ptr(), float(a), y.numel(), _stream()))
    return y


def adam_step(p, g, m, v, sumsq_acc, max_norm, gscale, lr, beta1, beta2, eps, step, zero_grad=False):
    fn = _lib.hip().stem_adam_step_zero if zero_grad else _lib.hip().stem_adam_step
    _chk(fn(p.data_ptr(), g.data_ptr(), m.data_ptr(), v.data_ptr(), p.numel(), _ptr(sumsq_acc),
            max_norm, gscale, lr, beta1, beta2, eps, step, _stream()))


def adam_step_bmax(p, g, m, v, sumsq_acc, max_norm, gscale, lr, beta1, beta2, eps, step, bmax, zero_grad=False):
    _chk(_lib.hip().stem_adam_step_bmax(p.data_ptr(), g.data_ptr(), m.data_ptr(), v.data_ptr(), p.numel(), _ptr(sumsq_acc),
                                        max_norm, gscale, lr, beta1, beta2, eps, step, int(bool(zero_grad)), bmax.data_ptr(), _stream()))


def adam_chunk():
    return int(_lib.hip().stem_adam_chunk())


def adam_step_dev(p, g, m, v, sumsq_acc, max_norm, gscale, lr_dev, beta1, beta2, eps, step_dev, scal_dev):
    _chk(_lib.hip().stem_adam_step_dev(p.data_ptr(), g.data_ptr(), m.data_ptr(), v.data_ptr(), p.numel(), _ptr(sumsq_acc),
                                       max_norm, gscale, lr_dev.data_ptr(), beta1, beta2, eps, step_dev.data_ptr(),
                                       scal_dev.data_ptr(), _stream()))


_M64 = 2 ** 64 - 1


def _noise_args(noise, seed, offset, epoch):
    if noise is not None:
        assert noise.is_cuda and noise.dtype == torch.float32
        return noise.data_ptr(), 0, 0, None, 0
    return None, int(seed) & _M64, int(offset) & _M64, (None if epoch is None else epoch.data_ptr()), (0 if epoch is None else NOISE_EPOCH_STRIDE)


def prior_prologue(yc, yd, residual, training, with_t_hat, noise=None, seed=0, offset=0, epoch=None, records=None):
    B, Cc, H, W = yc.shape
    dev = yc.device
    he_in, target = empty_nhwc(B, 2 * Cc, H, W, dev), empty_nhwc(B, Cc, H, W, dev)
    t_hat = empty_nhwc(B, Cc, H, W, dev) if with_t_hat else None
    y_hat = empty_nhwc(B, Cc, H, W, dev) if with_t_hat else None
    if noise is not None:
        assert nhwc_ld(noise) == Cc
    nptr, sd, off, ep, stride = _noise_args(noise, seed, offset, epoch)
    q_in = q_t = None
    if records is not None:
        q_in = records["in"] = qrec_for(B * H * W * Cc // 4, dev)
        if with_t_hat:
            q_t = records["t_hat"] = qrec_for(B * H * W * Cc // 4, dev)
    _chk(_lib.hip().stem_prior_prologue(yc.data_ptr(), nhwc_ld(yc), yd.data_ptr(), nhwc_ld(yd), he_in.data_ptr(), 2 * Cc, target.data_ptr(),
                                        _ptr(t_hat), _ptr(y_hat), nptr, sd, off, ep, stride, B * H * W, Cc, int(bool(residual)),
                                        int(bool(training)), _ptr(q_in), _ptr(q_t), _stream()))
    return he_in, target, t_hat, y_hat


def rate_partials(n):
    return int(_lib.hip().stem_rate_partials(n))


def eb_forward_train(z, pack, coef, noise=None, seed=0, offset=0, epoch=None, bound=1e-9, record=False):
    B, Cc, H, W = z.shape
    z_hat, lik, dlik = (empty_nhwc(B, Cc, H, W, z.device) for _ in range(3))
    part = torch.empty(rate_partials(z.numel()), dtype=torch.float64, device=z.device)
    if noise is not None:
        assert nhwc_ld(noise) == Cc
    nptr, sd, off, ep, stride = _noise_args(noise, seed, offset, epoch)
    if record:
        q = qrec_for(z.numel(), z.device)
        _chk(_lib.hip().stem_eb_forward_train_rec(z.data_ptr(), nhwc_ld(z), pack.data_ptr(), nptr, sd, off, ep, stride, z_hat.data_ptr(),
                                                  lik.data_ptr(), dlik.data_ptr(), part.data_ptr(), B * H * W, Cc, bound, coef, q.data_ptr(),
                                                  _stream()))
        return z_hat, lik, dlik, part, q
    _chk(_lib.hip().stem_eb_forward_train(z.data_ptr(), nhwc_ld(z), pack.data_ptr(), nptr, sd, off, ep, stride, z_hat.data_ptr(),
                                          lik.data_ptr(), dlik.data_ptr(), part.data_ptr(), B * H * W, Cc, bound, coef, _stream()))
    return z_hat, lik, dlik, part


def gc_forward_train(y, scales, means, coef, noise=None, seed=0, offset=0, epoch=None, scale_bound=0.11, lik_bound=1e-9, backward=None,
                     record=False):
    B, Cc, H, W = y.shape
    assert nhwc_ld(y) == Cc and nhwc_ld(scales) == nhwc_ld(means)
    out, lik, dlik = (empty_nhwc(B, Cc, H, W, y.device) for _ in range(3))
    part = torch.empty(rate_partials(y.numel()), dtype=torch.float64, device=y.device)
    if noise is not None:
        assert nhwc_ld(noise) == Cc
    nptr, sd, off, ep, stride = _noise_args(noise, seed, offset, epoch)
    if backward is not None:
        dsc, dmu = backward
        assert nhwc_ld(dsc) == nhwc_ld(dmu)
        q = qrec_for(B * H * W * Cc, y.device) if record else None
        _chk(_lib.hip().stem_gc_forward_backward_train(y.data_ptr(), scales.data_ptr(), means.data_ptr(), nhwc_ld(scales), nptr, sd, off, ep,
                                                       stride, out.data_ptr(), lik.data_ptr(), dlik.data_ptr(), part.data_ptr(), B * H * W, Cc,
                                                       scale_bound, lik_bound, coef, dsc.data_ptr(), dmu.data_ptr(), nhwc_ld(dsc), _ptr(q),
                                                       _stream()))
        return out, lik, dlik, part, q
    _chk(_lib.hip().stem_gc_forward_train(y.data_ptr(), scales.data_ptr(), means.data_ptr(), nhwc_ld(scales), nptr, sd, off, ep, stride,
                                          out.data_ptr(), lik.data_ptr(), dlik.data_ptr(), part.data_ptr(), B * H * W, Cc, scale_bound,
                                          lik_bound, coef, _stream()))
    return out, lik, dlik, part


def em_loss_finalize(part_y, part_z, scale, out3=None):
    if out3 is None:
        out3 = torch.empty(3, dtype=torch.float64, device=part_y.device)
    _chk(_lib.hip().stem_em_loss_finalize(part_y.data_ptr(), part_y.numel(), part_z.data_ptr(), part_z.numel(), float(scale),
                                          out3.data_ptr(), _stream()))
    return out3


def eb_forward_eval_rate(z, pack, medians, bound=1e-9):
    _require_cuda(z, pack, medians)
    B, Cc, H, W = z.shape
    ldz = nhwc_ld(z)
    assert ldz is not None, "eb_forward_eval_rate: z must be NHWC memory"
    assert pack.shape == (Cc, EB_NPARAM) and pack.is_contiguous() and medians.numel() == Cc and medians.is_contiguous()
    z_hat, lik = empty_nhwc(B, Cc, H, W, z.device), empty_nhwc(B, Cc, H, W, z.device)
    part = torch.empty(rate_partials(z.numel()), dtype=torch.float64, device=z.device)
    _chk(_lib.hip().stem_eb_forward_eval_rate(z.data_ptr(), ldz, pack.data_ptr(), medians.data_ptr(), z_hat.data_ptr(), lik.data_ptr(),
                                              part.data_ptr(), B * H * W, Cc, bound, _stream()))
    return z_hat, lik, part


def gc_forward_eval_rate(y, scales, means, scale_bound=0.11, lik_bound=1e-9):
    _require_cuda(y, scales, means)
    B, Cc, H, W = y.shape
    assert nhwc_ld(y) == Cc and scales.shape == y.shape and means.shape == y.shape
    ldsm = nhwc_ld(scales)
    assert ldsm is not None and ldsm == nhwc_ld(means)
    out, lik = empty_nhwc(B, Cc, H, W, y.device), empty_nhwc(B, Cc, H, W, y.device)
    part = torch.empty(rate_partials(y.numel()), dtype=torch.float64, device=y.device)
    _chk(_lib.hip().stem_gc_forward_eval_rate(y.data_ptr(), scales.data_ptr(), means.data_ptr(), ldsm, out.data_ptr(), lik.data_ptr(),
                                              part.data_ptr(), B * H * W, Cc, scale_bound, lik_bound, _stream()))
    return out, lik, part


def em_loss_accumulate(part_y, part_z, scale, acc4, weight=1.0, out3=None):
    assert acc4.is_cuda and acc4.dtype == torch.float64 and acc4.numel() == 4 and acc4.is_contiguous()
    for p in (part_y, part_z):
        assert p.dtype == torch.float64 and p.is_contiguous() and (p.is_cuda or p.numel() == 0)
    if out3 is None:
        out3 = torch.empty(3, dtype=torch.float64, device=acc4.device)
    assert out3.is_cuda and out3.dtype == torch.float64 and out3.numel() == 3 and out3.is_contiguous()
    _chk(_lib.hip().stem_em_loss_accumulate(part_y.data_ptr() if part_y.numel() else 0, part_y.numel(),
                                            part_z.data_ptr() if part_z.numel() else 0, part_z.numel(), float(scale), float(weight),
                                            out3.data_ptr(), acc4.data_ptr(), _stream()))
    return out3


def eb_aux_loss_grad(quantiles, pack, target, dq_out, loss_out=None, accumulate=False):
    if loss_out is None:
        loss_out = torch.empty(1, dtype=torch.float32, device=quantiles.device)
    _chk(_lib.hip().stem_eb_aux_loss_grad(quantiles.data_ptr(), pack.data_ptr(), target.data_ptr(), loss_out.data_ptr(),
                                          _ptr(dq_out), quantiles.shape[0], int(bool(accumulate)), _stream()))
    return loss_out


EBF_MAX_FILTERS, EBF_MAX_WIDTH, EBF_MAX_NPARAM = 6, 8, 433


def _ebf_filters(filters):
    f = tuple(int(v) for v in filters)
    return ((C.c_int * len(f))(*f) if f else None), len(f)


def ebf_in_caps(filters):
    f = tuple(int(v) for v in filters)
    return len(f) <= EBF_MAX_FILTERS and all(1 <= v <= EBF_MAX_WIDTH for v in f)


@functools.lru_cache(maxsize=None)
def _ebf_layout(f):
    if not ebf_in_caps(f):
        raise ValueError(f"filters={f} is outside the caps of the general bottleneck kernels: at most {EBF_MAX_FILTERS} filters, "
                         f"widths 1 .. {EBF_MAX_WIDTH}")
    widths = (1, *f, 1)
    out, off = [], 0
    for i in range(len(f) + 1):
        groups = [("_matrix", widths[i + 1] * widths[i]), ("_bias", widths[i + 1])] + ([("_factor", widths[i + 1])] if i < len(f) else [])
        for name, n in groups:
            out.append((f"{name}{i:d}", off, n))
            off += n
    return tuple(out), off


def ebf_layout(filters):
    return list(_ebf_layout(tuple(int(v) for v in filters))[0])


def ebf_nparam(filters):
    return _ebf_layout(tuple(int(v) for v in filters))[1]


def ebf_tensor_names(filters):
    return [name for name, _, _ in ebf_layout(filters)]


def ebf_pack(tensors, filters):
    ts = [t.detach().contiguous() for t in tensors]
    _require_cuda(*ts)
    layout = ebf_layout(filters)
    if len(ts) != len(layout) or any(t.numel() != ts[0].shape[0] * n for t, (_, _, n) in zip(ts, layout)):
        raise ValueError(f"ebf_pack: filters={tuple(filters)} takes {len(layout)} tensors of {[n for _, _, n in layout]} floats per channel")
    Cc = ts[0].shape[0]
    pack = torch.empty((Cc, ebf_nparam(filters)), device=ts[0].device, dtype=torch.float32)
    fa, nf = _ebf_filters(filters)
    _chk(_lib.hip().stem_ebf_pack(_ptr_array(ts), fa, nf, pack.data_ptr(), Cc, _stream()))
    return pack


def ebf_unpack_grads(dpack, grads, filters, accumulate=False):
    _require_cuda(dpack, *grads)
    layout = ebf_layout(filters)
    Cc = dpack.shape[0]
    if len(grads) != len(layout) or any(not g.is_contiguous() or g.numel() != Cc * n for g, (_, _, n) in zip(grads, layout)):
        raise ValueError(f"ebf_unpack_grads: filters={tuple(filters)} takes {len(layout)} contiguous tensors")
    if tuple(dpack.shape) != (Cc, ebf_nparam(filters)) or not dpack.is_contiguous():
        raise ValueError(f"ebf_unpack_grads: dpack must be a dense [C, {ebf_nparam(filters)}] tensor")
    fa, nf = _ebf_filters(filters)
    _chk(_lib.hip().stem_ebf_unpack_grads(dpack.data_ptr(), _ptr_array(grads), fa, nf, Cc, 1 if accumulate else 0, _stream()))


def _ebf_check_pack(pack, filters, Cc):
    if tuple(pack.shape) != (Cc, ebf_nparam(filters)) or not pack.is_contiguous():
        raise ValueError(f"pack must be a dense [{Cc}, {ebf_nparam(filters)}] tensor for filters={tuple(filters)}, got {tuple(pack.shape)}")


def ebf_forward(z, pack, filters, medians=None, noise=None, bound=1e-9):
    _require_cuda(z, pack, medians, noise)
    B, Cc, H, W = z.shape
    _ebf_check_pack(pack, filters, Cc)
    ldz = nhwc_ld(z)
    if ldz is None:
        raise ValueError("ebf_forward: z must have NHWC memory")
    z_hat, lik = empty_nhwc(B, Cc, H, W, z.device), empty_nhwc(B, Cc, H, W, z.device)
    mode = 0 if noise is not None else 1
    if noise is not None and (tuple(noise.shape) != tuple(z.shape) or nhwc_ld(noise) != Cc):
        raise ValueError("ebf_forward: noise must be a dense NHWC tensor of z's shape")
    if medians is not None and (medians.numel() != Cc or not medians.is_contiguous()):
        raise ValueError("ebf_forward: medians must be a contiguous [C] tensor")
    fa, nf = _ebf_filters(filters)
    _chk(_lib.hip().stem_ebf_forward(z.data_ptr(), ldz, _ptr(noise), pack.data_ptr(), _ptr(medians), fa, nf, z_hat.data_ptr(),
                                     lik.data_ptr(), B, H, W, Cc, mode, bound, _stream()))
    return z_hat, lik


def ebf_backward(z_hat, pack, dlik, filters, dzhat_in=None, bound=1e-9, want_dz=True, want_dpack=True, dz_out=None, dpack_out=None):
    _require_cuda(z_hat, pack, dlik, dzhat_in, dz_out, dpack_out)
    B, Cc, H, W = z_hat.shape
    _ebf_check_pack(pack, filters, Cc)
    for t in (z_hat, dlik, dzhat_in, dz_out):
        if t is not None and (tuple(t.shape) != (B, Cc, H, W) or nhwc_ld(t) != Cc):
            raise ValueError("ebf_backward: z_hat, dlik, dzhat_in and dz must be dense NHWC tensors of one shape")
    dz = (dz_out if dz_out is not None else empty_nhwc(B, Cc, H, W, z_hat.device)) if want_dz else None
    dpack = (dpack_out if dpack_out is not None else torch.empty_like(pack)) if want_dpack else None
    if dpack is not None:
        _ebf_check_pack(dpack, filters, Cc)
    fa, nf = _ebf_filters(filters)
    _chk(_lib.hip().stem_ebf_backward(z_hat.data_ptr(), pack.data_ptr(), dlik.data_ptr(), _ptr(dzhat_in), fa, nf, _ptr(dz), _ptr(dpack),
                                      B, H, W, Cc, bound, _stream()))
    return dz, dpack


def ebf_aux_loss_grad(quantiles, pack, target, filters, dq_out, loss_out=None, accumulate=False):
    _require_cuda(quantiles, pack, target, dq_out, loss_out)
    Cc = quantiles.shape[0]
    _ebf_check_pack(pack, filters, Cc)
    if quantiles.numel() != 3 * Cc or not quantiles.is_contiguous() or (dq_out is not None and (dq_out.numel() != 3 * Cc or not dq_out.is_contiguous())):
        raise ValueError("ebf_aux_loss_grad: quantiles and dq_out must be contiguous [C, 1, 3] tensors")
    if loss_out is None:
        loss_out = torch.empty(1, dtype=torch.float32, device=quantiles.device)
    fa, nf = _ebf_filters(filters)
    _chk(_lib.hip().stem_ebf_aux_loss_grad(quantiles.data_ptr(), pack.data_ptr(), target.data_ptr(), fa, nf, loss_out.data_ptr(),
                                           _ptr(dq_out), Cc, int(bool(accumulate)), _stream()))
    return loss_out
```

### spatiotemporalentropymodel_amd/optim.py

```python
from __future__ import annotations

import torch

from . import functional as F
from .layers import bump_weight_epoch, join_wgrad_stream


BACKWARD_ORDER = ("EPM.", "context_prediction.", "TPM.", "HD.", "entropy_bottleneck.", "HE.")


def backward_layout_key(name):
    for i, pre in enumerate(BACKWARD_ORDER):
        if name.startswith(pre):
            return (i, name)
    return (len(BACKWARD_ORDER), name)


class FlatParameters:

    def __init__(self, named_params, layout_key=None):
        self.names = [n for n, _ in named_params]
        self.params = [p for _, p in named_params]
        dev = self.params[0].device
        order = sorted(range(len(self.params)), key=(lambda i: layout_key(self.names[i])) if layout_key else None)
        self.offsets, off = [0] * len(self.params), 0
        for i in order:
            self.offsets[i] = off
            off += (self.params[i].numel() + 3) // 4 * 4
        self.numel = off
        self.data = torch.zeros(off, device=dev, dtype=torch.float32)
        self.grad = torch.zeros(off, device=dev, dtype=torch.float32)
        for p, o in zip(self.params, self.offsets):
            n = p.numel()
            self.data[o:o + n].copy_(p.detach().reshape(-1))
            p.data = self.data[o:o + n].view(p.shape)
            p._flat_grad_view = self.grad[o:o + n].view(p.shape)
            p.grad = p._flat_grad_view
        bump_weight_epoch(self.params)

    def restore(self, data):
        self.data.copy_(data)
        bump_weight_epoch(self.params)

    def zero_grad(self):
        join_wgrad_stream()
        if self.grad.is_cuda:
            F.zero_bytes(self.grad)
        else:
            self.grad.zero_()
        for p in self.params:
            p.grad = p._flat_grad_view


class FusedClipAdam(torch.optim.Optimizer):

    def __init__(self, flat: FlatParameters, lr, max_norm=None, betas=(0.9, 0.999), eps=1e-8):
        defaults = dict(lr=float(lr), betas=tuple(betas), eps=float(eps), weight_decay=0, amsgrad=False, maximize=False,
                        foreach=None, capturable=False, differentiable=False, fused=None)
        super().__init__(flat.params, defaults)
        self.flat, self.max_norm = flat, max_norm
        self.m = torch.zeros_like(flat.data)
        self.v = torch.zeros_like(flat.data)
        self.t = 0
        self._sumsq = F.sumsq_accumulator(flat.data.device)
        self._dev = None

    lr = property(lambda self: self.param_groups[0]["lr"])
    betas = property(lambda self: self.param_groups[0]["betas"])
    eps = property(lambda self: self.param_groups[0]["eps"])

    def zero_grad(self, set_to_none=False):
        self.flat.zero_grad()

    def grad_norm(self):
        join_wgrad_stream()
        self._sumsq[:1].zero_()
        F.sumsq(self.flat.grad, self._sumsq)
        return self._sumsq[0].sqrt().reshape(())

    def enable_device_state(self):
        if self._dev is None:
            dev = self.flat.data.device
            self._dev = {"step": torch.zeros(1, dtype=torch.int64, device=dev), "lr": torch.zeros(1, dtype=torch.float32, device=dev),
                         "scal": torch.zeros(2, dtype=torch.float32, device=dev), "lr_host": None}
        self.sync_device_state()
        return self

    def sync_device_state(self):
        d = self._dev
        if d is None:
            return
        d["step"].fill_(self.t)
        lr = float(self.param_groups[0]["lr"])
        if d["lr_host"] != lr:
            d["lr"].fill_(lr)
            d["lr_host"] = lr

    def step(self, closure=None, *, grad_scale: float = 1.0, norm_is_current: bool = False, zero_grad: bool = False,
             block_max: bool = False):
        loss = None
        if closure is not None:
            with torch.enable_grad():
                loss = closure()
        join_wgrad_stream()
        self.t += 1
        g = self.param_groups[0]
        use_clip = self.max_norm is not None and self.max_norm > 0
        if use_clip and not norm_is_current:
            self._sumsq[:1].zero_()
            F.sumsq(self.flat.grad, self._sumsq)
        if self._dev is not None:
            d = self._dev
            if not torch.cuda.is_current_stream_capturing():
                if d["lr_host"] != float(g["lr"]):
                    d["lr"].fill_(float(g["lr"]))
                    d["lr_host"] = float(g["lr"])
            F.adam_step_dev(self.flat.data, self.flat.grad, self.m, self.v, self._sumsq if use_clip else None,
                            float(self.max_norm) if use_clip else 0.0, float(grad_scale), d["lr"], g["betas"][0], g["betas"][1],
                            float(g["eps"]), d["step"], d["scal"])
        elif block_max:
            if getattr(self, "block_maxima", None) is None:
                ch = F.adam_chunk()
                self.block_maxima = torch.empty(4 * ((self.flat.data.numel() + ch - 1) // ch), device=self.flat.data.device, dtype=torch.float32)
            F.adam_step_bmax(self.flat.data, self.flat.grad, self.m, self.v, self._sumsq if use_clip else None,
                             float(self.max_norm) if use_clip else 0.0, float(grad_scale), float(g["lr"]), g["betas"][0], g["betas"][1],
                             float(g["eps"]), self.t, self.block_maxima, zero_grad=zero_grad)
        else:
            F.adam_step(self.flat.data, self.flat.grad, self.m, self.v, self._sumsq if use_clip else None,
                        float(self.max_norm) if use_clip else 0.0, float(grad_scale), float(g["lr"]), g["betas"][0], g["betas"][1],
                        float(g["eps"]), self.t, zero_grad=zero_grad)
        if self._dev is None:
            gs = float(grad_scale)
            F.tape_bind_floats(lambda: (float(self.max_norm) if use_clip else 0.0, gs, float(g["lr"]), float(g["betas"][0]),
                                        float(g["betas"][1]), float(g["eps"])))
        bump_weight_epoch(self.flat.params)
        return loss

    def _views(self, buf):
        return [buf[o:o + p.numel()].view(p.shape) for p, o in zip(self.flat.params, self.flat.offsets)]

    def _sync_state(self):
        self.state.clear()
        if self.t == 0:
            return
        for p, m, v in zip(self.flat.params, self._views(self.m), self._views(self.v)):
            self.state[p] = {"step": torch.tensor(float(self.t)), "exp_avg": m, "exp_avg_sq": v}

    def state_dict(self):
        self._sync_state()
        return super().state_dict()

    def load_state_dict(self, state_dict):
        groups = state_dict["param_groups"]
        if len(groups) != 1 or len(groups[0]["params"]) != len(self.flat.params):
            raise ValueError(f"FusedClipAdam: expected one parameter group of {len(self.flat.params)} tensors "
                             f"(utils.py:104-135 order: sorted parameter names), got {[len(g['params']) for g in groups]}")
        super().load_state_dict(state_dict)
        steps = set()
        self.m.zero_()
        self.v.zero_()
        for p, m, v in zip(self.flat.params, self._views(self.m), self._views(self.v)):
            st = self.state.get(p)
            if not st:
                continue
            m.copy_(st["exp_avg"])
            v.copy_(st["exp_avg_sq"])
            steps.add(int(float(st["step"])))
        if len(steps) > 1:
            raise ValueError(f"FusedClipAdam: parameters carry different step counts {sorted(steps)}; the fused step keeps one")
        self.t = steps.pop() if steps else 0
        self._sync_state()
        self.sync_device_state()


def clip_grad_norm_(optimizers, max_norm, tensors=None):
    join_wgrad_stream()
    optimizers = [o for o in optimizers if o is not None]
    bufs = list(tensors) if tensors is not None else [o.flat.grad for o in optimizers]
    acc = optimizers[0]._sumsq
    acc[:1].zero_()
    for g in bufs:
        F.sumsq(g, acc)
    for g in bufs:
        F.clip_scale(g, acc, max_norm)
    return acc[0].sqrt().reshape(())


def configure_optimizers(net, args, fused=True, max_norm=1.0):
    named = list(net.named_parameters())
    main = sorted([(n, p) for n, p in named if not n.endswith(".quantiles") and p.requires_grad], key=lambda t: t[0])
    aux = sorted([(n, p) for n, p in named if n.endswith(".quantiles") and p.requires_grad], key=lambda t: t[0])
    assert len(main) + len(aux) == len([1 for _, p in named if p.requires_grad])
    if not fused:
        return (torch.optim.Adam((p for _, p in main), lr=args.learning_rate),
                torch.optim.Adam((p for _, p in aux), lr=args.aux_learning_rate))
    return (FusedClipAdam(FlatParameters(main, layout_key=backward_layout_key), args.learning_rate, max_norm=max_norm),
            FusedClipAdam(FlatParameters(aux), args.aux_learning_rate, max_norm=None))
```

### spatiotemporalentropymodel_amd/tape.py

```python
from __future__ import annotations

import ctypes as C
import struct
import warnings

import torch
from torch.utils._python_dispatch import TorchDispatchMode

from . import _lib
from . import functional as F


class TapeRefused(RuntimeError):
    """the schedule cannot be replayed faithfully (it is not static, or it contains device work a tape does not hold)"""


def _pattern(ty, value):
    if ty is C.c_float:
        return struct.unpack("<d", struct.pack("<fI", float(value), 0))[0]
    return float(value)


class LaunchTape:

    def __init__(self):
        self.entries = []
        self.keep = []
        self.in_py = 0
        self.foreign = []
        self.problems = []
        self.float_bindings = {}
        self._bound_now = {}
        self._native = None
        self._segments = None

    def add_call(self, name, fn, args):
        sig = _lib._HIP_SIG[name]
        addr = C.cast(fn, C.c_void_p).value
        if not _lib.hip().stem_tape_entry_recordable(addr):
            self.problems.append(f"{name} is not in the library's table of recordable entry points (csrc/tape_entries.inc)")
            return
        if len(args) != len(sig):
            self.problems.append(f"{name}: {len(args)} arguments for a prototype of {len(sig)}")
            return
        kinds, ivals, fvals, keep = [], [], [], []
        isptr = [ty is C.c_void_p for ty in sig]
        for a, ty in zip(args, sig):
            if ty is C.c_float or ty is C.c_double:
                kinds.append(1 if ty is C.c_float else 2); ivals.append(0); fvals.append(_pattern(ty, a))
                continue
            kinds.append(0); fvals.append(0.0)
            if a is None:
                ivals.append(0)
            elif isinstance(a, int):
                ivals.append(a)
            elif isinstance(a, (C.Array, C.Structure)):
                ivals.append(C.addressof(a)); keep.append(a)
            elif isinstance(a, C.c_void_p):
                ivals.append(a.value or 0)
            else:
                self.problems.append(f"{name}: argument of type {type(a).__name__} is not recordable (pass addresses as integers)")
                return
        self.entries.append(("call", name, addr, kinds, ivals, fvals, keep, isptr))

    def bind_floats(self, provider):
        i = len(self.entries) - 1
        if i < 0 or self.entries[i][0] != "call":
            raise RuntimeError("tape_bind_floats: no recorded call to bind to")
        nf = sum(1 for k in self.entries[i][3] if k != 0)
        if len(provider()) != nf:
            raise RuntimeError(f"tape_bind_floats: {self.entries[i][1]} has {nf} float arguments, the provider returns {len(provider())}")
        self.float_bindings[i] = provider

    def _float_patterns(self, i):
        x = self.entries[i]
        sig = _lib._HIP_SIG[x[1]]
        ftys = [ty for ty in sig if ty is C.c_float or ty is C.c_double]
        return [_pattern(ty, v) for ty, v in zip(ftys, self.float_bindings[i]())]

    def refresh_floats(self):
        lib, n = _lib.hip(), 0
        for i in self.float_bindings:
            now = self._float_patterns(i)
            old = self._bound_now[i]
            if now != old and [struct.pack("<d", v) for v in now] != [struct.pack("<d", v) for v in old]:
                for pos, (a, b) in enumerate(zip(now, old)):
                    if struct.pack("<d", a) != struct.pack("<d", b):
                        _lib.check(lib.stem_tape_set_farg(self._native, self.native_index[i], pos, a))
                        n += 1
                self._bound_now[i] = now
        return n

    def finalize(self, second: "LaunchTape"):
        a, b = self.entries, second.entries
        if len(a) != len(b) or any(x[0] != y[0] or (x[0] == "call" and x[1] != y[1]) for x, y in zip(a, b)):
            raise TapeRefused("LaunchTape: two consecutive steps issued different launch sequences -- the schedule is not static")
        if self.problems or second.problems:
            raise TapeRefused("LaunchTape: " + "; ".join(sorted(set(self.problems + second.problems))))
        if self.foreign or second.foreign:
            ops = sorted(set(self.foreign + second.foreign))
            raise TapeRefused("LaunchTape: the step runs torch operators on device memory that a replay would drop: " + ", ".join(ops))
        if set(self.float_bindings) != set(second.float_bindings):
            raise TapeRefused("LaunchTape: the two recordings bound different launches to float providers")
        lib = _lib.hip()
        nat = lib.stem_tape_create()
        segs, lo = [], 0
        ndyn = 0
        self.native_index = []
        for ei, (x, y) in enumerate(zip(a, b)):
            if x[0] != "call":
                self.native_index.append(-1)
            if x[0] == "py":
                hi = lib.stem_tape_length(nat)
                if hi > lo:
                    segs.append((lo, hi))
                segs.append(x)
                lo = hi
                continue
            if x[0] == "wait":
                _lib.check(min(0, lib.stem_tape_add_wait(nat, x[1], x[2])))
            elif x[0] == "evrec":
                _lib.check(min(0, lib.stem_tape_add_event(nat, x[1], x[2], 0)))
            elif x[0] == "evwait":
                _lib.check(min(0, lib.stem_tape_add_event(nat, x[2], x[1], 1)))
            else:
                _, name, addr, kinds, iv, fv, _keep, isptr = x
                self.native_index.append(lib.stem_tape_length(nat))
                deltas = [0] * len(iv)
                bound = ei in self.float_bindings
                if bound:
                    cur = self._float_patterns(ei)
                    self._bound_now[ei] = cur
                    it = iter(cur)
                    fv = [next(it) if k != 0 else 0.0 for k in kinds]
                for i, (k, va, vb, fa, fb) in enumerate(zip(kinds, iv, y[4], fv, y[5])):
                    if k != 0:
                        if not bound and struct.pack('<d', fa) != struct.pack('<d', fb):
                            raise TapeRefused(f"LaunchTape: float argument {i} of {name} changed between two steps ({fa} -> {fb}) and no "
                                              "provider is bound to it (functional.tape_bind_floats)")
                    elif va != vb:
                        if isptr[i]:
                            continue
                        if vb < va:
                            raise TapeRefused(f"LaunchTape: integer argument {i} of {name} went from {va} to {vb} between two steps: not a step counter")
                        deltas[i] = vb - va
                        ndyn += 1
                n = len(iv)
                _lib.check(min(0, lib.stem_tape_add_call(nat, addr, n, (C.c_ubyte * n)(*kinds), (C.c_longlong * n)(*iv), (C.c_double * n)(*fv),
                                                         (C.c_longlong * n)(*deltas))))
        hi = lib.stem_tape_length(nat)
        if hi > lo:
            segs.append((lo, hi))
        self._native, self._segments, self.dynamic_args = nat, segs, ndyn
        return self

    def pointer_slots(self, address):
        out = []
        for x, ni in zip(self.entries, self.native_index):
            if x[0] != "call":
                continue
            pos = 0
            for k, v, isp in zip(x[3], x[4], x[7]):
                if k != 0:
                    continue
                if isp and v == address:
                    out.append((ni, pos))
                pos += 1
        return out

    def set_pointer(self, slots, address):
        lib = _lib.hip()
        for ni, pos in slots:
            _lib.check(lib.stem_tape_set_iarg(self._native, ni, pos, address))

    def replay(self, n):
        lib = _lib.hip()
        for seg in self._segments:
            if len(seg) == 2:
                rc = lib.stem_tape_replay(self._native, seg[0], seg[1], n)
                if rc != 0:
                    raise RuntimeError(f"LaunchTape: entry {-rc - 1} ({self.entries[-rc - 1][1]}) failed: {(lib.stem_last_error() or b'').decode()}")
            else:
                _, fn, stream = seg
                with F.on_stream(stream):
                    fn()

    def __len__(self):
        return len(self.entries)

    def __del__(self):
        try:
            if self._native:
                _lib.hip().stem_tape_destroy(self._native)
        except Exception:
            pass


class _RecordingLibrary:

    def __init__(self, lib, tape):
        self._lib, self._tape, self._cache = lib, tape, {}

    def __getattr__(self, name):
        w = self._cache.get(name)
        if w is not None:
            return w
        fn = getattr(self._lib, name)
        if (name not in _lib._HIP_SIG or name in _lib._RESTYPE or name.startswith("stem_tape_") or name.startswith("stem_tuning")
                or name.startswith("stem_stream_flag_")):
            return fn
        tape = self._tape

        def recorded(*args, _fn=fn, _name=name):
            rc = _fn(*args)
            if rc == 0:
                tape.add_call(_name, _fn, args)
            return rc
        self._cache[name] = recorded
        return recorded


class _ForeignOpGuard(TorchDispatchMode):

    BENIGN = frozenset("""empty empty_like empty_strided new_empty new_empty_strided view _unsafe_view reshape _reshape_alias
        as_strided slice select narrow permute transpose t unsqueeze squeeze expand expand_as detach alias unbind split
        split_with_sizes chunk view_as flatten unflatten movedim diagonal record_stream is_pinned size stride numel dim
        is_contiguous storage_offset sym_size sym_stride sym_numel sym_storage_offset is_same_size _has_compatible_shallow_copy_type
        set_ resize_ lift_fresh _to_copy_meta is_nonzero_meta""".split())

    def __init__(self, tape, is_device=None):
        super().__init__()
        self.tape = tape
        self.is_device = is_device or (lambda t: t.is_cuda)

    def __torch_dispatch__(self, func, types, args=(), kwargs=None):
        out = func(*args, **(kwargs or {}))
        if self.tape.in_py == 0:
            name = getattr(getattr(func, "overloadpacket", func), "__name__", str(func))
            if name not in self.BENIGN:
                import torch.utils._pytree as pytree
                leaves = pytree.tree_leaves((args, kwargs or {}, out))
                if any(isinstance(t, torch.Tensor) and self.is_device(t) for t in leaves):
                    self.tape.foreign.append(f"aten::{name}")
        return out


class recording:

    _ALLOC = ("empty", "zeros", "empty_like", "zeros_like", "empty_strided")

    def __init__(self, tape, keep_allocations):
        self.tape, self.keep_alloc = tape, keep_allocations

    def __enter__(self):
        if F._TAPE is not None:
            raise RuntimeError("a launch tape is already recording")
        self._real = _lib.hip()
        _lib._hip = _RecordingLibrary(self._real, self.tape)
        F._TAPE = self.tape
        self._guard = _ForeignOpGuard(self.tape)
        self._guard.__enter__()
        self._saved = {}
        if self.keep_alloc:
            keep = self.tape.keep
            for n in self._ALLOC:
                real = getattr(torch, n)
                self._saved[n] = real

                def held(*a, _real=real, **kw):
                    t = _real(*a, **kw)
                    keep.append(t)
                    return t
                setattr(torch, n, held)
            self._clone = torch.Tensor.clone

            def clone(t, *a, _real=self._clone, **kw):
                r = _real(t, *a, **kw)
                keep.append(r)
                return r
            torch.Tensor.clone = clone
        return self.tape

    def __exit__(self, *exc):
        self._guard.__exit__(*exc)
        _lib._hip = self._real
        F._TAPE = None
        for n, real in self._saved.items():
            setattr(torch, n, real)
        if self.keep_alloc:
            torch.Tensor.clone = self._clone
        return False


class TapedPFrameStep:

    WARMUP = 2

    def __init__(self, fused):
        self.fused = fused
        self.refused = None
        self._reset(None)

    def _reset(self, key):
        self.key, self.calls, self.tape, self.first = key, 0, None, None
        self.replays = 0
        self.refused = None

    taped = property(lambda self: self.tape is not None)

    def _counters(self):
        f = self.fused
        objs = [(f.opt, "t"), (f.aux_opt, "t"), (f.stem.entropy_bottleneck, "_noise_offset"), (f.stem.gaussian_conditional, "_noise_offset")]
        return [(o, a) for o, a in objs if hasattr(o, a)]

    def _refuse(self, why):
        self.refused, self.tape, self.first = str(why), None, None
        warnings.warn(f"TapedPFrameStep: running the ordinary schedule instead of a launch tape -- {why}", RuntimeWarning, stacklevel=3)

    def _key(self, y_cur, y_cond, num_pixels, grad_scale, reducer):
        f = self.fused
        clip = tuple(bool(o.max_norm is not None and o.max_norm > 0) for o in (f.opt, f.aux_opt))
        return (tuple(y_cur.shape), tuple(y_cond.shape), tuple(y_cur.stride()), tuple(y_cond.stride()), y_cur.dtype, y_cond.dtype, y_cur.device,
                int(num_pixels), float(grad_scale), id(reducer), F.cur_stream(y_cur.device).cuda_stream, clip, bool(f.clear_grad_in_adam),
                bool(f.adam_block_max), bool(f.overwrite_grads))

    def step(self, y_cur, y_cond, num_pixels, grad_scale=1.0, reducer=None):
        key = self._key(y_cur, y_cond, num_pixels, grad_scale, reducer)
        if key != self.key:
            self._reset(key)
        f = self.fused
        if self.refused is not None:
            return f.step(y_cur, y_cond, num_pixels, grad_scale, reducer)
        if self.calls == 0:
            if f.opt._dev is not None or f.aux_opt._dev is not None:
                self._refuse("the optimiser keeps its step count / learning rate in device memory (enable_device_state)")
                return f.step(y_cur, y_cond, num_pixels, grad_scale, reducer)
            for name, t in (("y_cur", y_cur), ("y_cond", y_cond)):
                if F.nhwc_ld(t) is None and not t.is_contiguous():
                    self._refuse(f"{name} is neither NHWC nor contiguous: the schedule would convert it with a torch copy")
                    return f.step(y_cur, y_cond, num_pixels, grad_scale, reducer)
        self.calls += 1
        if self.calls <= self.WARMUP:
            return f.step(y_cur, y_cond, num_pixels, grad_scale, reducer)
        if self.calls == self.WARMUP + 1:
            self.in_cur = torch.empty_strided(y_cur.size(), y_cur.stride(), dtype=y_cur.dtype, device=y_cur.device)
            self.in_cond = torch.empty_strided(y_cond.size(), y_cond.stride(), dtype=y_cond.dtype, device=y_cond.device)
            if self.in_cur.stride() != y_cur.stride() or self.in_cond.stride() != y_cond.stride():
                self._refuse("the input latents' strides cannot be reproduced in a recorded buffer")
                return f.step(y_cur, y_cond, num_pixels, grad_scale, reducer)
            self.in_cur.copy_(y_cur)
            self.in_cond.copy_(y_cond)
            self.first = LaunchTape()
            before = [getattr(o, a) for o, a in self._counters()]
            try:
                with recording(self.first, keep_allocations=True):
                    self.result = f.step(self.in_cur, self.in_cond, num_pixels, grad_scale, reducer)
            except BaseException:
                self._reset(None)
                raise
            self.deltas = [getattr(o, a) - b for (o, a), b in zip(self._counters(), before)]
            return self.result
        if self.calls == self.WARMUP + 2:
            second = LaunchTape()
            try:
                with recording(second, keep_allocations=False):
                    res = f.step(y_cur, y_cond, num_pixels, grad_scale, reducer)
            except BaseException:
                self._reset(None)
                raise
            try:
                self.tape = self.first.finalize(second)
            except TapeRefused as e:
                self._refuse(e)
                return res
            self.replays = 1
            self.cur_slots = self.tape.pointer_slots(self.in_cur.data_ptr())
            self.cond_slots = self.tape.pointer_slots(self.in_cond.data_ptr())
            y_hat = self.result[0]["y_hat"]
            self.yhat_slots = self.tape.pointer_slots(y_hat.data_ptr())
            self.yhat_bufs = [y_hat, torch.empty_like(y_hat)] if (self.cond_slots and self.yhat_slots) else None
            self._weights_key = f.eng._weights_key()
            return res
        if f.eng._weights_key() != self._weights_key:
            f.eng._pack_key = None
            f.eng.ensure_packed(split=False)
        if self.cur_slots:
            self.tape.set_pointer(self.cur_slots, y_cur.data_ptr())
        else:
            self.in_cur.copy_(y_cur)
        result = self.result
        if self.yhat_bufs is not None:
            out = self.yhat_bufs[1] if y_cond.data_ptr() == self.yhat_bufs[0].data_ptr() else self.yhat_bufs[0]
            self.tape.set_pointer(self.cond_slots, y_cond.data_ptr())
            self.tape.set_pointer(self.yhat_slots, out.data_ptr())
            if out is not self.yhat_bufs[0]:
                result = (dict(self.result[0], y_hat=out),) + tuple(self.result[1:])
        else:
            self.in_cond.copy_(y_cond)
        self.tape.refresh_floats()
        self.replays += 1
        self.tape.replay(self.replays)
        for (o, a), d in zip(self._counters(), self.deltas):
            setattr(o, a, getattr(o, a) + d)
        f.after_replay()
        self._weights_key = f.eng._weights_key()
        return result

    def packs_are_current(self):
        if self.tape is not None and self.replays > 1:
            self.fused.eng._pack_key = self._weights_key

    def finish(self):
        self.fused.finish()
```

### spatiotemporalentropymodel_amd/trainer.py

```python
from __future__ import annotations

import contextlib
import math
import os

import torch

from . import config as _config
from . import functional as F
from .layers import join_wgrad_stream


SCHEDULE_DEFAULTS = {"STEM_STREAM_PRIO": "latents=0,side=-1,compute=-1", "STEM_STREAM_CUMASK": "latents=block:160"}


def tuned_schedule(device):
    for k, v in SCHEDULE_DEFAULTS.items():
        os.environ.setdefault(k, v)
    F.make_stream(device, "side")
    if "compute" in (F._STREAM_PRIO or {}):
        return torch.cuda.stream(F.make_stream(device, "compute"))
    return contextlib.nullcontext()


class LatentPrefetcher:

    def __init__(self, imodel, ahead=1):
        self.imodel, self.ahead = imodel, int(ahead)
        self._stream = None
        self._frames = self._ys = self._events = None
        self._next = 0
        self._nxt = None

    def _enqueue_into(self, frames, ys, events, t):
        dev = frames[t].device
        if self._stream is None or self._stream.device != dev:
            self._stream = F.make_stream(dev, "latents")
        with F.on_stream(self._stream), torch.no_grad():
            ys[t] = self.imodel.getY(frames[t])
            events[t] = torch.cuda.Event()
            events[t].record(self._stream)

    def _enqueue(self, t):
        self._enqueue_into(self._frames, self._ys, self._events, t)

    def start(self, frames, frames_ready=False, next_frames=None):
        frames = list(frames) if not isinstance(frames, list) else frames
        n = len(frames)
        adopted = 0
        if self._nxt is not None and (self._nxt["frames"] is frames or
                                      (len(self._nxt["frames"]) == n and all(a is b for a, b in zip(self._nxt["frames"], frames)))):
            self._ys, self._events, adopted = self._nxt["ys"], self._nxt["events"], self._nxt["n"]
        else:
            self._ys, self._events = [None] * n, [None] * n
        self._frames = frames
        self._nxt = None
        if next_frames is not None:
            nf = list(next_frames) if not isinstance(next_frames, list) else next_frames
            self._nxt = {"frames": nf, "ys": [None] * len(nf), "events": [None] * len(nf), "n": 0}
        dev = self._frames[0].device
        if self._stream is None or self._stream.device != dev:
            self._stream = F.make_stream(dev, "latents")
        if not frames_ready:
            F.stream_wait(self._stream, F.cur_stream(dev))
        self._next = adopted
        while self._next < n and self._next <= self.ahead:
            self._enqueue(self._next)
            self._next += 1
        return self

    def get(self, t):
        n = len(self._frames)
        while self._next < n and self._next <= t + self.ahead:
            self._enqueue(self._next)
            self._next += 1
        if self._nxt is not None and self._next >= n:
            want = min(t + self.ahead + 2 - n, self.ahead + 1, len(self._nxt["frames"]))
            while self._nxt["n"] < want:
                self._enqueue_into(self._nxt["frames"], self._nxt["ys"], self._nxt["events"], self._nxt["n"])
                self._nxt["n"] += 1
        cur = F.cur_stream(self._frames[t].device)
        cur.wait_event(self._events[t])
        y, yq = self._ys[t]
        y.record_stream(cur)
        yq.record_stream(cur)
        return y, yq


class LazyScalar:

    def __init__(self, value, event, scale=1.0, sqrt=False):
        self._v, self._e, self._scale, self._sqrt = value, event, scale, sqrt

    def tensor(self):
        cur = F.cur_stream(self._v.device)
        cur.wait_event(self._e)
        self._v.record_stream(cur)
        v = self._v.reshape(())
        return (v.sqrt() if self._sqrt else v) * self._scale if (self._sqrt or self._scale != 1.0) else v

    def __float__(self):
        return float(self.tensor())


class FusedPFrameStep:
    def __init__(self, stem, optimizer, aux_optimizer):
        self.stem, self.opt, self.aux_opt = stem, optimizer, aux_optimizer
        self.eng = stem.engine()
        eb = stem.entropy_bottleneck
        if eb.quantiles.grad is None or getattr(eb.quantiles, "_flat_grad_view", None) is None:
            raise ValueError("FusedPFrameStep needs the flat-buffer optimisers of optim.configure_optimizers(fused=True)")
        self._aux_loss = torch.zeros(1, dtype=torch.float32, device=eb.quantiles.device)
        self._grad_clean = False
        self.clear_grad_in_adam = True
        self.overwrite_grads = _config.runtime().trainer_overwrite_grads
        self.adam_block_max = _config.runtime().adam_block_max
        self._aux_stream = self.eng.side_stream(eb.quantiles.device) or F.make_stream(eb.quantiles.device, "side")
        self._aux_pending = False
        self._done_event = torch.cuda.Event()

    def step(self, y_cur, y_cond, num_pixels, grad_scale=1.0, reducer=None):
        stem, opt, aux_opt, eng = self.stem, self.opt, self.aux_opt, self.eng
        eb = stem.entropy_bottleneck
        overwrite = bool(self.overwrite_grads)
        if overwrite or (self._grad_clean and opt._dev is None):
            for p in opt.flat.params:
                p.grad = p._flat_grad_view
        else:
            opt.flat.zero_grad()
        coef = -1.0 / (math.log(2.0) * num_pixels)
        y_hat, lik_y, lik_z, k = eng.forward(y_cur, y_cond, True, rate_coef=(coef, -1.0 / num_pixels))
        eng.accumulate_grads = not overwrite
        try:
            eng.backward(k, k["dlik_y"], k["dlik_z"])
        finally:
            eng.accumulate_grads = True
        if reducer is not None:
            F.tape_py(reducer.finish if hasattr(reducer, "finish") else reducer.all_reduce)
        join_wgrad_stream()
        main = F.cur_stream(y_hat.device)
        if self._aux_pending:
            F.stream_wait(main, self._aux_stream)
            self._aux_pending = False
        F.sumsq(opt.flat.grad, opt._sumsq, overwrite=True)
        clean = opt._dev is None and self.clear_grad_in_adam and not overwrite
        use_bmax = opt._dev is None and eng.use_fx3 and self.adam_block_max
        opt.step(grad_scale=grad_scale, norm_is_current=True, zero_grad=clean, block_max=use_bmax)
        self._grad_clean = clean
        F.stream_wait(self._aux_stream, main)
        with F.on_stream(self._aux_stream):
            gn_copy = F.copy_d2d(torch.empty_like(opt._sumsq[:1]), opt._sumsq[:1])
            pack = F.eb_pack(eb._tensors14())
            F.eb_aux_loss_grad(eb.quantiles.detach(), pack, eb.target, eb.quantiles._flat_grad_view, loss_out=self._aux_loss)
            eb.quantiles.grad = eb.quantiles._flat_grad_view
            aux_opt.step()
            aux_copy = F.copy_d2d(torch.empty_like(self._aux_loss), self._aux_loss)
            done = self._done_event
            F.event_record(done, self._aux_stream)
        self._aux_pending = True
        eng.ensure_packed(block_max=(opt.block_maxima, opt.flat.data) if use_bmax else None)
        loss3 = k["loss3"]
        out = {"y_hat": y_hat, "likelihoods": {"y": lik_y, "z": lik_z}}
        oc = {"y_bpp_loss": loss3[0], "z_bpp_loss": loss3[1], "loss": loss3[2]}
        return out, oc, LazyScalar(aux_copy, done), LazyScalar(gn_copy, done, scale=grad_scale, sqrt=True)

    def after_replay(self):
        from .layers import bump_weight_epoch
        bump_weight_epoch(self.opt.flat.params)
        self._aux_pending = True

    def finish(self):
        if self._aux_pending:
            F.stream_wait(F.cur_stream(self._aux_loss.device), self._aux_stream)
            self._aux_pending = False


def subsample_septuplet(images, rand):
    if rand <= 0.25:
        return images[0:7:2]
    if rand <= 0.50:
        return images[0:7:3]
    if rand <= 0.75:
        return images[0:7:6]
    return images


class SeptupletTrainer:

    def __init__(self, imodel, stem, optimizer, aux_optimizer, *, route="taped", prefetch=True, ahead=1, reducer=None, grad_scale=1.0,
                 criterion=None, rng=None):
        import random
        self.imodel, self.stem, self.opt, self.aux_opt = imodel, stem, optimizer, aux_optimizer
        self.route, self.reducer, self.grad_scale, self.criterion = route, reducer, float(grad_scale), criterion
        self.rng = rng or random.Random(0)
        self.step_fn = None
        if route in ("taped", "fused"):
            self.step_fn = FusedPFrameStep(stem, optimizer, aux_optimizer)
            if route == "taped":
                from .tape import TapedPFrameStep
                self.step_fn = TapedPFrameStep(self.step_fn)
        elif route != "generic":
            raise ValueError(f"SeptupletTrainer: unknown route {route!r}")
        elif criterion is None:
            raise ValueError("SeptupletTrainer: the generic route needs the criterion module")
        self.prefetch = LatentPrefetcher(imodel, ahead=ahead) if prefetch else None
        self.on_step = None

    def train_septuplet(self, images, rand=None, next_images=None, frames_ready=True):
        frames = list(subsample_septuplet(list(images), self.rng.random() if rand is None else rand))
        num_pixels = frames[0].shape[0] * frames[0].shape[-2] * frames[0].shape[-1]
        if self.prefetch is not None:
            self.prefetch.start(frames, frames_ready=frames_ready, next_frames=next_images)
            ys = None
            y_cond = self.prefetch.get(0)[1]
        else:
            with torch.no_grad():
                ys = [self.imodel.getY(f) for f in frames]
            y_cond = ys[0][1]
        log = []
        for t in range(1, len(frames)):
            y_cur = self.prefetch.get(t)[0] if self.prefetch is not None else ys[t][0]
            if self.step_fn is not None:
                out, oc, aux, gn = self.step_fn.step(y_cur, y_cond, num_pixels, grad_scale=self.grad_scale, reducer=self.reducer)
            else:
                from .selfcheck import p_frame_step
                out, oc, aux, gn = p_frame_step(self.imodel, self.stem, self.criterion, self.opt, self.aux_opt, frames[t], y_cond,
                                                grad_scale=self.grad_scale, reducer=self.reducer, y_cur=y_cur)
            y_cond = out["y_hat"]
            log.append((oc, aux, gn))
            if self.on_step is not None:
                self.on_step(t, out, oc, aux, gn)
        return log

    def finish(self):
        if self.step_fn is not None:
            self.step_fn.finish()

    def validate(self, loader, **kw):
        self.finish()
        if hasattr(self.step_fn, "packs_are_current"):
            self.step_fn.packs_are_current()
        if kw.get("prefetch", True) is True and self.prefetch is not None:
            if getattr(self, "_val_prefetch", None) is None:
                self._val_prefetch = LatentPrefetcher(self.imodel, ahead=self.prefetch.ahead)
            kw["prefetch"] = self._val_prefetch
        elif kw.get("prefetch", True) is True:
            kw["prefetch"] = False
        if self.criterion is not None:
            kw.setdefault("criterion", self.criterion)
        return validate(self.imodel, self.stem, loader, **kw)


def image_step(model, criterion, optimizer, aux_optimizer, x, clip_max_norm=1.0):
    from .layers import to_nchw
    from .optim import clip_grad_norm_
    optimizer.zero_grad()
    aux_optimizer.zero_grad()
    out_net = model(x)
    if F.nhwc_ld(out_net["x_hat"]) is not None and not out_net["x_hat"].is_contiguous():
        out_net = dict(out_net, x_hat=to_nchw(out_net["x_hat"]))
    out_criterion = criterion(out_net, x)
    out_criterion["loss"].backward()
    grad_norm = None
    if clip_max_norm > 0:
        if hasattr(optimizer, "flat"):
            grad_norm = clip_grad_norm_((optimizer, aux_optimizer), clip_max_norm)
        else:
            join_wgrad_stream()
            grad_norm = torch.nn.utils.clip_grad_norm_(model.parameters(), clip_max_norm)
    optimizer.step()
    aux_loss = model.aux_loss()
    aux_loss.backward()
    aux_optimizer.step()
    return out_criterion, aux_loss, grad_norm


@contextlib.contextmanager
def _eval_modes(*models):
    modes = [(mod, mod.training) for m in models for mod in m.modules()]
    try:
        for m in models:
            m.eval()
        yield
    finally:
        for mod, flag in modes:
            mod.training = flag


@contextlib.contextmanager
def _noise_offsets_kept(*models):
    kept = [(mod, mod._noise_offset) for m in models for mod in m.modules() if hasattr(mod, "_noise_offset")]
    try:
        yield
    finally:
        for mod, off in kept:
            mod._noise_offset = off


def _stem_route(stem, route):
    if route not in (None, "fused", "generic"):
        raise ValueError(f"validate: unknown route {route!r}")
    if route == "generic":
        return None
    if route is None and DEFAULT_VALIDATION_ROUTE != "fused":
        return None
    if route is None and tuple(stem.entropy_bottleneck.filters) != (3, 3, 3, 3):
        return None
    return stem.engine()


DEFAULT_VALIDATION_ROUTE = "fused"


def validate(imodel, stem, loader, *, criterion=None, route=None, prefetch=True, lr_scheduler=None, max_items=None):
    eng = _stem_route(stem, route)
    if eng is None and criterion is None:
        from .losses import EMLoss
        criterion = EMLoss()
    pf = prefetch if isinstance(prefetch, LatentPrefetcher) else (LatentPrefetcher(imodel) if prefetch else None)
    acc = None
    with torch.no_grad(), _eval_modes(imodel, stem), _noise_offsets_kept(imodel, stem):
        for n, images in enumerate(loader):
            if max_items is not None and n >= max_items:
                break
            frames = list(images)
            if len(frames) < 2:
                raise ValueError(f"validate: loader item {n} has {len(frames)} frame(s); a P step needs two")
            B, _, H, W = frames[0].shape
            if acc is None:
                acc = torch.zeros(4, dtype=torch.float64, device=frames[0].device)
            if pf is not None:
                pf.start(frames, frames_ready=True)
                y_cond = pf.get(0)[1]
            else:
                y_cond = imodel.getY(frames[0])[1]
            for t in range(1, len(frames)):
                y_cur = pf.get(t)[0] if pf is not None else imodel.getY(frames[t])[0]
                if eng is not None:
                    y_cond = eng.eval_rate(y_cur, y_cond, B * H * W, acc=acc, weight=float(B))[0]
                else:
                    out = stem(y_cur, y_cond)
                    oc = criterion(out, frames[t])
                    y_cond = out["y_hat"]
                    acc += float(B) * torch.stack([oc["y_bpp_loss"].double().reshape(()), oc["z_bpp_loss"].double().reshape(()),
                                                   oc["loss"].double().reshape(()), torch.ones((), dtype=torch.float64, device=acc.device)])
    if acc is None:
        raise ValueError("validate: the loader is empty")
    a = acc.cpu().tolist()
    res = {"y_bpp_loss": a[0] / a[3], "z_bpp_loss": a[1] / a[3], "loss": a[2] / a[3], "count": a[3]}
    if lr_scheduler is not None:
        lr_scheduler.step(res["loss"])
    return res


def _nchw_x_hat(out_net):
    from .layers import to_nchw
    if F.nhwc_ld(out_net["x_hat"]) is not None and not out_net["x_hat"].is_contiguous():
        return dict(out_net, x_hat=to_nchw(out_net["x_hat"]))
    return out_net


def _mean_dict(sums, cnt):
    vals = torch.stack([v.double().reshape(()) for v in sums.values()]).cpu().tolist()
    return {k: v / cnt for k, v in zip(sums, vals)}


def validate_pixel(model_i, model_p, loaders, criterion, *, criterion_rd=None):
    first = loaders[0] if isinstance(loaders, (list, tuple)) and len(loaders) else None
    roi = isinstance(loaders, (list, tuple)) and not (isinstance(first, (list, tuple)) and len(first) and torch.is_tensor(first[0]))
    if roi and criterion_rd is None:
        from .losses import RateDistortionLoss
        criterion_rd = RateDistortionLoss()
    from .losses import quality2lambda
    results = []
    with torch.no_grad(), _eval_modes(model_i, model_p), _noise_offsets_kept(model_i, model_p):
        for loader in (loaders if roi else [loaders]):
            sums, cnt = {}, 0
            for item in loader:
                images, qmap = item if roi else (item, None)
                lmbdamap = quality2lambda(qmap) if roi else None
                x_cond = None
                for idx, x in enumerate(images):
                    if roi:
                        out = _nchw_x_hat(model_i(x, qmap) if idx == 0 else model_p(x, x_cond, qmap))
                        oc = criterion(out, x, lmbdamap)
                        vals = {"loss": oc["loss"], "mse_loss": oc["mse_loss"], "bpp_loss": oc["bpp_loss"], "mse": criterion_rd(out, x)["mse_loss"]}
                    else:
                        out = _nchw_x_hat(model_i(x) if idx == 0 else model_p(x, x_cond))
                        oc = criterion(out, x)
                        vals = {"loss": oc["loss"], "mse_loss": oc["mse_loss"], "bpp_loss": oc["bpp_loss"]}
                    x_cond = out["x_hat"]
                    for k, v in vals.items():
                        sums[k] = v.detach().double() if k not in sums else sums[k] + v.detach().double()
                    cnt += 1
            if not cnt:
                raise ValueError("validate_pixel: an empty loader")
            results.append(_mean_dict(sums, cnt))
    return results if roi else results[0]


def validate_image(model, loader, criterion):
    sums, cnt = {}, 0
    with torch.no_grad(), _eval_modes(model), _noise_offsets_kept(model):
        for x in loader:
            oc = criterion(_nchw_x_hat(model(x)), x)
            vals = {"loss": oc["loss"], "bpp_loss": oc["bpp_loss"], "mse_loss": oc["mse_loss"], "aux_loss": model.aux_loss()}
            for k, v in vals.items():
                sums[k] = v.detach().double() if k not in sums else sums[k] + v.detach().double()
            cnt += 1
    if not cnt:
        raise ValueError("validate_image: an empty loader")
    return _mean_dict(sums, cnt)


def fit(trainer, train_loader, test_loader, lr_scheduler, epochs, *, start_epoch=0, start_iterations=0, validate_every=20000, save=None,
        save_every_epochs=2, on_validation=None):
    from .utils import save_checkpoint
    state = {"iterations": int(start_iterations), "best": float("inf"), "epoch": int(start_epoch), "log": []}

    def checkpoint(name):
        if save is None:
            return
        trainer.finish()
        save_checkpoint({"epoch": state["epoch"], "iterations": state["iterations"], "state_dict": trainer.stem.state_dict(),
                         "optimizer": trainer.opt.state_dict(), "aux_optimizer": trainer.aux_opt.state_dict(),
                         "lr_scheduler": lr_scheduler.state_dict()}, filename=save + name)

    def after_step(*step):
        if user_hook is not None:
            user_hook(*step)
        state["iterations"] += 1
        if validate_every and state["iterations"] % validate_every == 0:
            res = trainer.validate(test_loader, lr_scheduler=lr_scheduler)
            best = res["loss"] < state["best"]
            state["log"].append((state["epoch"], state["iterations"], res["loss"]))
            if best:
                state["best"] = res["loss"]
                checkpoint(f"checkpoint_best_epoch{state['epoch']}.pth.tar")
            if on_validation is not None:
                on_validation(state["epoch"], state["iterations"], res, best)

    user_hook = trainer.on_step
    trainer.on_step = after_step
    try:
        for epoch in range(int(start_epoch), int(epochs)):
            state["epoch"] = epoch
            for images in train_loader:
                trainer.train_septuplet(images)
            if save_every_epochs and epoch % save_every_epochs == 0:
                checkpoint(f"checkpoint_epoch{epoch}.pth.tar")
    finally:
        trainer.on_step = user_hook
    trainer.finish()
    return {"iterations": state["iterations"], "best_loss": state["best"], "validations": state["log"]}


def resume_state(checkpoint, stem, optimizer, aux_optimizer, lr_scheduler):
    stem.load_state_dict(checkpoint["state_dict"])
    optimizer.load_state_dict(checkpoint["optimizer"])
    aux_optimizer.load_state_dict(checkpoint["aux_optimizer"])
    lr_scheduler.load_state_dict(checkpoint["lr_scheduler"])
    return checkpoint["epoch"] + 1, checkpoint["iterations"]
```

Baseline: 10180 frames/s.

## Split Adam step into ordered parameter-range launches overlapping next step's layers

Adds a range-based Adam kernel in a new tail library and plans the optimiser step as several launches over chunk ranges grouped by the layers that consume them. Each layer waits on a per-group tail event before its forward or input-grad pass, so early layers of the next step can start while later parameters are still being updated. This is meant to hide the serial optimiser tail behind compute. It adds more launches, more events and a new library to bind into the launch tape.

```diff
diff --git a/__graft_entry__.py b/__graft_entry__.py
--- a/__graft_entry__.py
+++ b/__graft_entry__.py
@@ -18,6 +18,7 @@
     _lib.rans()
     _lib.frameio()
     _lib.roiio()
+    _lib.tail()
 
 
 def smoke() -> None:
diff --git a/include/stem_tail.h b/include/stem_tail.h
--- /dev/null
+++ b/include/stem_tail.h
@@ -0,0 +1,22 @@
+#ifndef STEM_TAIL_H
+#define STEM_TAIL_H
+#include <stddef.h>
+#include <stdint.h>
+
+#define STEM_ADAM_MAX_RANGES 40
+
+#ifdef __cplusplus
+extern "C" {
+#endif
+
+int stem_adam_step_bmax_ranges(float *p, float *g, float *m, float *v, size_t n, const double *sumsq, float max_norm, float gscale,
+                               float lr, float beta1, float beta2, float eps, int step, int zero_grad, float *bmax,
+                               const int *ranges, int nranges, void *stream);
+
+const char *stem_tail_last_error(void);
+int stem_tail_entry_recordable(void *fn);
+
+#ifdef __cplusplus
+}
+#endif
+#endif
diff --git a/spatiotemporalentropymodel_amd/_lib.py b/spatiotemporalentropymodel_amd/_lib.py
--- a/spatiotemporalentropymodel_amd/_lib.py
+++ b/spatiotemporalentropymodel_amd/_lib.py
@@ -11,12 +11,14 @@
 RANS_SO = os.environ.get("STEM_RANS_LIBRARY") or os.path.join(_PKG, "libstem_rans.so")
 
 FRAMEIO_SO = os.path.join(_PKG, "libstem_frameio.so")
+TAIL_SO = os.path.join(_PKG, "libstem_tail.so")
 ROIIO_SO = os.path.join(_PKG, "libstem_roiio.so")
 DP_SO = os.environ.get("STEM_DP_LIBRARY") or os.path.join(_PKG, "libstem_dp.so")
 _hip = None
 _rans = None
 _dp = None
 _frameio = None
+_tail = None
 _roiio = None
 
 
@@ -43,6 +45,8 @@
 _HIP_EBF_PROTO, _HIP_EBF_SIG, _ = _tables("stem_eb_filters.h")
 _HIP_GDN1_PROTO, _HIP_GDN1_SIG, _ = _tables("stem_gdn1.h")
 _HIP_VALIDATION_PROTO, _HIP_VALIDATION_SIG, _ = _tables("stem_validation.h")
+_TAIL_PROTO, _TAIL_SIG, _ = _tables("stem_tail.h")
+_TAPE_SIG = {**_HIP_SIG, **{n: a for n, a in _TAIL_SIG.items() if not n.startswith("stem_tail_")}}
 _FRAMEIO_PROTO, _FRAMEIO_SIG, _ = _tables("stem_frameio.h")
 _ROIIO_PROTO, _ROIIO_SIG, _ = _tables("stem_roiio.h")
 _RANS_PROTO, _RANS_SIG, _RANS_RESTYPE = _tables("stem_rans.h")
@@ -107,6 +111,21 @@
     return _frameio
 
 
+def tail():
+    global _tail
+    if _tail is None:
+        if not os.path.exists(TAIL_SO):
+            raise StemLibraryError(f"{TAIL_SO} is missing: build it with `python -c 'import __graft_entry__ as g; g.build()'` "
+                                   "(hipcc --offload-arch=gfx950).  There is no fallback for the ordered optimiser tail's kernel.")
+        _tail = _bind(C.CDLL(TAIL_SO), _TAIL_PROTO)
+    return _tail
+
+
+def check_tail(rc: int):
+    if rc != 0:
+        raise RuntimeError((tail().stem_tail_last_error() or b"").decode() or f"libstem_tail error {rc}")
+
+
 def check_frameio(rc: int):
     if rc != 0:
         raise RuntimeError((frameio().stem_frameio_last_error() or b"").decode() or f"libstem_frameio error {rc}")
@@ -169,6 +188,10 @@
     return sorted(_HIP_VALIDATION_SIG)
 
 
+def declared_tail_symbols():
+    return sorted(_TAIL_SIG)
+
+
 def declared_frameio_symbols():
     return sorted(_FRAMEIO_SIG)
 
diff --git a/spatiotemporalentropymodel_amd/config.py b/spatiotemporalentropymodel_amd/config.py
--- a/spatiotemporalentropymodel_amd/config.py
+++ b/spatiotemporalentropymodel_amd/config.py
@@ -25,6 +25,7 @@
     engine_split_pack: bool = True
     engine_pack_pair: bool = True
     engine_branch: bool = True
+    engine_tail_ordered: bool = True
     stream_prio: str = ""
     stream_cumask: str = ""
     dp_threaded: int = 3
@@ -46,6 +47,7 @@
     "layers_f16x3_maxpix": "STEM_LAYERS_F16X3_MAXPIX", "layers_wide_minpix": "STEM_LAYERS_WIDE_MINPIX",
     "adam_block_max": "STEM_ADAM_BLOCK_MAX", "trainer_overwrite_grads": "STEM_TRAINER_OVERWRITE_GRADS", "engine_overlap": "STEM_ENGINE_OVERLAP",
     "engine_split_pack": "STEM_ENGINE_SPLIT_PACK", "engine_pack_pair": "STEM_ENGINE_PACK_PAIR", "engine_branch": "STEM_ENGINE_BRANCH",
+    "engine_tail_ordered": "STEM_ENGINE_TAIL_ORDERED",
     "stream_prio": "STEM_STREAM_PRIO", "stream_cumask": "STEM_STREAM_CUMASK", "dp_min_bytes": "STEM_DP_MIN_BYTES", "dp_threaded": "STEM_DP_THREADED",
     "dist_backend": "STEM_DIST_BACKEND", "dist_single": "STEM_DIST_SINGLE", "pin_ranks": "STEM_PIN_RANKS",
     "ar_persistent": "STEM_AR_PERSISTENT", "ar_stepwise": "STEM_AR_STEPWISE",
diff --git a/spatiotemporalentropymodel_amd/csrc/adam_chunk.h b/spatiotemporalentropymodel_amd/csrc/adam_chunk.h
--- /dev/null
+++ b/spatiotemporalentropymodel_amd/csrc/adam_chunk.h
@@ -0,0 +1,49 @@
+#pragma once
+#include "stem_common.h"
+
+namespace {
+
+__device__ __forceinline__ void adam_chunk_pass(float *p, float *g, float *m, float *v, size_t n, const double *sumsq, float max_norm,
+                                                float gscale, float step_size, float b1, float b2, float inv_sqrt_bc2, float eps,
+                                                int zero_g, float *bmax, unsigned chunk)
+{
+    float coef = gscale;
+    if (max_norm > 0.f && sumsq) {
+        const float total = (float)sqrt(sumsq[0]) * gscale;
+        coef *= fminf(max_norm / (total + 1e-6f), 1.0f);
+    }
+    const size_t base = (size_t)chunk * STEM_ADAM_CHUNK;
+    float mx = 0.f;
+#pragma unroll 1
+    for (int k0 = 0; k0 < STEM_ADAM_CHUNK / 256; k0 += 4) {
+        float gi[4], mi[4], vi[4], pi[4];
+        size_t idx[4];
+#pragma unroll
+        for (int u = 0; u < 4; ++u) {
+            idx[u] = base + (size_t)(k0 + u) * 256 + threadIdx.x;
+            const bool ok = idx[u] < n;
+            const size_t j = ok ? idx[u] : 0;
+            gi[u] = ok ? g[j] : 0.f;
+            mi[u] = ok ? m[j] : 0.f;
+            vi[u] = ok ? v[j] : 0.f;
+            pi[u] = ok ? p[j] : 0.f;
+        }
+#pragma unroll
+        for (int u = 0; u < 4; ++u) {
+            if (idx[u] >= n) continue;
+            const float gs = gi[u] * coef;
+            if (zero_g) g[idx[u]] = 0.f;
+            const float mn = mi[u] + (gs - mi[u]) * (1.f - b1);
+            const float vn = vi[u] * b2 + (1.f - b2) * gs * gs;
+            m[idx[u]] = mn;
+            v[idx[u]] = vn;
+            const float pn = pi[u] - step_size * (mn / (sqrtf(vn) * inv_sqrt_bc2 + eps));
+            p[idx[u]] = pn;
+            mx = fmaxf(mx, fabsf(pn));
+        }
+    }
+    mx = wave_max(mx);
+    if ((threadIdx.x & 63) == 0) bmax[chunk * 4 + (threadIdx.x >> 6)] = mx;
+}
+
+}
diff --git a/spatiotemporalentropymodel_amd/csrc/optim.hip b/spatiotemporalentropymodel_amd/csrc/optim.hip
--- a/spatiotemporalentropymodel_amd/csrc/optim.hip
+++ b/spatiotemporalentropymodel_amd/csrc/optim.hip
@@ -1,4 +1,5 @@
 #include "stem_common.h"
+#include "adam_chunk.h"
 
 namespace {
 
@@ -62,43 +63,7 @@
                                                         float max_norm, float gscale, float step_size, float b1, float b2,
                                                         float inv_sqrt_bc2, float eps, int zero_g, float *bmax)
 {
-    float coef = gscale;
-    if (max_norm > 0.f && sumsq) {
-        const float total = (float)sqrt(sumsq[0]) * gscale;
-        coef *= fminf(max_norm / (total + 1e-6f), 1.0f);
-    }
-    const size_t base = (size_t)blockIdx.x * STEM_ADAM_CHUNK;
-    float mx = 0.f;
-#pragma unroll 1
-    for (int k0 = 0; k0 < STEM_ADAM_CHUNK / 256; k0 += 4) {
-        float gi[4], mi[4], vi[4], pi[4];
-        size_t idx[4];
-#pragma unroll
-        for (int u = 0; u < 4; ++u) {
-            idx[u] = base + (size_t)(k0 + u) * 256 + threadIdx.x;
-            const bool ok = idx[u] < n;
-            const size_t j = ok ? idx[u] : 0;
-            gi[u] = ok ? g[j] : 0.f;
-            mi[u] = ok ? m[j] : 0.f;
-            vi[u] = ok ? v[j] : 0.f;
-            pi[u] = ok ? p[j] : 0.f;
-        }
-#pragma unroll
-        for (int u = 0; u < 4; ++u) {
-            if (idx[u] >= n) continue;
-            const float gs = gi[u] * coef;
-            if (zero_g) g[idx[u]] = 0.f;
-            const float mn = mi[u] + (gs - mi[u]) * (1.f - b1);
-            const float vn = vi[u] * b2 + (1.f - b2) * gs * gs;
-            m[idx[u]] = mn;
-            v[idx[u]] = vn;
-            const float pn = pi[u] - step_size * (mn / (sqrtf(vn) * inv_sqrt_bc2 + eps));
-            p[idx[u]] = pn;
-            mx = fmaxf(mx, fabsf(pn));
-        }
-    }
-    mx = wave_max(mx);
-    if ((threadIdx.x & 63) == 0) bmax[blockIdx.x * 4 + (threadIdx.x >> 6)] = mx;
+    adam_chunk_pass(p, g, m, v, n, sumsq, max_norm, gscale, step_size, b1, b2, inv_sqrt_bc2, eps, zero_g, bmax, blockIdx.x);
 }
 
 __global__ void adam_prepare_kernel(long long *step, const float *lr, float b1, float b2, float *scal)
diff --git a/spatiotemporalentropymodel_amd/csrc/tail.hip b/spatiotemporalentropymodel_amd/csrc/tail.hip
--- /dev/null
+++ b/spatiotemporalentropymodel_amd/csrc/tail.hip
@@ -0,0 +1,85 @@
+#include <stdarg.h>
+
+#include <algorithm>
+#include <iterator>
+
+#include "../../include/stem_tail.h"
+#include "adam_chunk.h"
+#include "tape_contract.h"
+
+static thread_local char g_err[512] = "";
+void stem_set_error(const char *fmt, ...)
+{
+    va_list ap;
+    va_start(ap, fmt);
+    vsnprintf(g_err, sizeof(g_err), fmt, ap);
+    va_end(ap);
+}
+STEM_EXPORT const char *stem_tail_last_error(void) { return g_err; }
+
+namespace {
+
+constexpr int ADAM_MAXRANGES = STEM_ADAM_MAX_RANGES;
+struct AdamRangeTable {
+    unsigned c0[ADAM_MAXRANGES];
+    unsigned wg0[ADAM_MAXRANGES + 1];
+    int n;
+};
+__global__ __launch_bounds__(256) void adam_bmax_ranges_kernel(float *p, float *g, float *m, float *v, size_t n, const double *sumsq,
+                                                               float max_norm, float gscale, float step_size, float b1, float b2,
+                                                               float inv_sqrt_bc2, float eps, int zero_g, float *bmax,
+                                                               const AdamRangeTable tab)
+{
+    int r = 0;
+    while (r + 1 < tab.n && blockIdx.x >= tab.wg0[r + 1]) ++r;
+    adam_chunk_pass(p, g, m, v, n, sumsq, max_norm, gscale, step_size, b1, b2, inv_sqrt_bc2, eps, zero_g, bmax,
+                    tab.c0[r] + (blockIdx.x - tab.wg0[r]));
+}
+
+#define STEM_TAPE_ENTRY(name) \
+    static_assert(tape_recordable(&name), #name ": prototype outside the launch tape's calling contract (csrc/tape.hip)");
+#include "tape_entries_tail.inc"
+#undef STEM_TAPE_ENTRY
+
+#define STEM_TAPE_ENTRY(name) reinterpret_cast<const void *>(&name),
+const void *const kRecordable[] = {
+#include "tape_entries_tail.inc"
+};
+#undef STEM_TAPE_ENTRY
+
+}
+
+STEM_EXPORT int stem_tail_entry_recordable(void *fn)
+{
+    return std::find(std::begin(kRecordable), std::end(kRecordable), (const void *)fn) != std::end(kRecordable) ? 1 : 0;
+}
+
+STEM_EXPORT int stem_adam_step_bmax_ranges(float *p, float *g, float *m, float *v, size_t n, const double *sumsq, float max_norm,
+                                           float gscale, float lr, float beta1, float beta2, float eps, int step, int zero_grad,
+                                           float *bmax, const int *ranges, int nranges, void *stream)
+{
+    STEM_CHECK_ARG(p && g && m && v && bmax && step >= 1, "stem_adam_step_bmax_ranges: bad arguments");
+    STEM_CHECK_ARG(nranges >= 0 && nranges <= ADAM_MAXRANGES && (ranges || nranges == 0),
+                   "stem_adam_step_bmax_ranges: %d ranges (at most %d)", nranges, ADAM_MAXRANGES);
+    if (n == 0) return 0;
+    const size_t nchunks = cdivz(n, STEM_ADAM_CHUNK);
+    AdamRangeTable tab;
+    memset(&tab, 0, sizeof(tab));
+    unsigned wgs = 0;
+    for (int r = 0; r < nranges; ++r) {
+        const int c0 = ranges[2 * r], c1 = ranges[2 * r + 1];
+        STEM_CHECK_ARG(c0 >= 0 && c0 <= c1 && (size_t)c1 <= nchunks, "stem_adam_step_bmax_ranges: range %d = [%d, %d) outside the %zu chunks",
+                       r, c0, c1, nchunks);
+        if (c0 == c1) continue;
+        tab.c0[tab.n] = (unsigned)c0;
+        tab.wg0[tab.n++] = wgs;
+        wgs += (unsigned)(c1 - c0);
+    }
+    tab.wg0[tab.n] = wgs;
+    if (wgs == 0) return 0;
+    const double bc1 = 1.0 - pow((double)beta1, step), bc2 = 1.0 - pow((double)beta2, step);
+    hipLaunchKernelGGL(adam_bmax_ranges_kernel, dim3(wgs), dim3(256), 0, (hipStream_t)stream, p, g, m, v, n, sumsq, max_norm, gscale,
+                       (float)(lr / bc1), beta1, beta2, (float)(1.0 / sqrt(bc2)), eps, zero_grad, bmax, tab);
+    STEM_LAUNCH_CHECK("adam_bmax_ranges");
+    return 0;
+}
diff --git a/spatiotemporalentropymodel_amd/csrc/tape.hip b/spatiotemporalentropymodel_amd/csrc/tape.hip
--- a/spatiotemporalentropymodel_amd/csrc/tape.hip
+++ b/spatiotemporalentropymodel_amd/csrc/tape.hip
@@ -5,10 +5,10 @@
 #include <vector>
 
 #include "stem_common.h"
+#include "tape_contract.h"
 
 namespace {
 
-constexpr int TAPE_MAXI = 40, TAPE_MAXF = 6;
 enum { TAPE_CALL = 0, TAPE_WAIT = 1, TAPE_EVENT_RECORD = 2, TAPE_EVENT_WAIT = 3 };
 
 struct TapeEntry {
@@ -55,17 +55,6 @@
 }
 const auto kCallers = make_callers(std::make_index_sequence<TAPE_MAXI + 1>{});
 
-static_assert(TAPE_MAXF <= 8, "SSE arguments beyond xmm7 go to the stack and would interleave with the integer overflow area");
-template <class T>
-constexpr bool tape_int_class = (std::is_integral<T>::value || std::is_enum<T>::value || std::is_pointer<T>::value) && sizeof(T) <= 8;
-template <class T>
-constexpr bool tape_sse_class = std::is_same<T, float>::value || std::is_same<T, double>::value;
-template <class... A>
-constexpr bool tape_recordable(int (*)(A...))
-{
-    constexpr int ni = (0 + ... + (tape_int_class<A> ? 1 : 0)), nf = (0 + ... + (tape_sse_class<A> ? 1 : 0));
-    return ni + nf == (int)sizeof...(A) && ni <= TAPE_MAXI && nf <= TAPE_MAXF;
-}
 #define STEM_TAPE_ENTRY(name) \
     static_assert(tape_recordable(&name), #name ": prototype outside the launch tape's calling contract (csrc/tape.hip)");
 #include "tape_entries.inc"
diff --git a/spatiotemporalentropymodel_amd/csrc/tape_contract.h b/spatiotemporalentropymodel_amd/csrc/tape_contract.h
--- /dev/null
+++ b/spatiotemporalentropymodel_amd/csrc/tape_contract.h
@@ -0,0 +1,20 @@
+#pragma once
+#include <type_traits>
+
+namespace {
+
+constexpr int TAPE_MAXI = 40, TAPE_MAXF = 6;
+
+static_assert(TAPE_MAXF <= 8, "SSE arguments beyond xmm7 go to the stack and would interleave with the integer overflow area");
+template <class T>
+constexpr bool tape_int_class = (std::is_integral<T>::value || std::is_enum<T>::value || std::is_pointer<T>::value) && sizeof(T) <= 8;
+template <class T>
+constexpr bool tape_sse_class = std::is_same<T, float>::value || std::is_same<T, double>::value;
+template <class... A>
+constexpr bool tape_recordable(int (*)(A...))
+{
+    constexpr int ni = (0 + ... + (tape_int_class<A> ? 1 : 0)), nf = (0 + ... + (tape_sse_class<A> ? 1 : 0));
+    return ni + nf == (int)sizeof...(A) && ni <= TAPE_MAXI && nf <= TAPE_MAXF;
+}
+
+}
diff --git a/spatiotemporalentropymodel_amd/csrc/tape_entries_tail.inc b/spatiotemporalentropymodel_amd/csrc/tape_entries_tail.inc
--- /dev/null
+++ b/spatiotemporalentropymodel_amd/csrc/tape_entries_tail.inc
@@ -0,0 +1,2 @@
+STEM_TAPE_ENTRY(stem_adam_step_bmax_ranges)
+STEM_TAPE_ENTRY(stem_tail_entry_recordable)
diff --git a/spatiotemporalentropymodel_amd/engine.py b/spatiotemporalentropymodel_amd/engine.py
--- a/spatiotemporalentropymodel_amd/engine.py
+++ b/spatiotemporalentropymodel_amd/engine.py
@@ -56,6 +56,8 @@
         self._slabs = {}
         self.pending = None
         self.lane = 0
+        self.tail_event = None
+        self.tail_group = 0
 
     def fx3_eligible(self):
         return self.kind == "conv" and not self.masked and _layers.f16x3_same_shape(self.stride, self.R, self.pad, self.C, self.K)
@@ -137,6 +139,8 @@
 
     def forward(self, a, act=F.ACT_NONE, out=None, planes=False):
         self.eng.ensure_packed()
+        if self.tail_event is not None:
+            self.eng._wait_tail(self)
         face, m = self.faces[0], self.mod
         epi = F.GEN_EPI_LRELU if act == F.ACT_LRELU else F.GEN_EPI_BIAS
         if face.kind == "gen":
@@ -155,6 +159,8 @@
         return self.forward(_Act(x), act, out=out).x
 
     def input_grad(self, dy, xact=None, planes=False, x_shape=None):
+        if self.tail_event is not None:
+            self.eng._wait_tail(self)
         face = self.faces[1]
         epi = F.GEN_EPI_DACT if xact is not None else F.GEN_EPI_BIAS
         if face.kind == "gen":
@@ -255,6 +261,23 @@
     d.bmax, d.b0 = maxima.data_ptr(), off // ch
     d.nb = (off + numel - 1) // ch - d.b0 + 1
     return True
+
+
+def tail_chunk_ranges(tensors, numel, ch, ngroups):
+    nch = (numel + ch - 1) // ch
+    cgroup = [ngroups] * nch
+    for off, n, gi in tensors:
+        for c in range(off // ch, (off + max(n, 1) - 1) // ch + 1):
+            cgroup[c] = min(cgroup[c], gi)
+    out = [[] for _ in range(ngroups)]
+    c = 0
+    while c < nch:
+        gi, c1 = cgroup[c], c
+        while c1 < nch and cgroup[c1] == gi:
+            c1 += 1
+        out[0 if gi == ngroups else gi].append((c, c1))
+        c = c1
+    return out
 
 
 def _grad_of(p):
@@ -291,6 +314,9 @@
         self._fwd32_pack_event = None
         self.accumulate_grads = True
         self._events = {}
+        self._tail_cache = None
+        self._tail_last = None
+        self._tail_waited = set()
         self._select_fx3()
 
     def _select_fx3(self):
@@ -361,6 +387,7 @@
             return
         if self._weights_key() == self._pack_key:
             return
+        self._drop_tail()
         have = [l.wp_fwd if l.faces[0].kind == "f32" else l.wp6_fwd for l in self.layers]
         if any(h is None or h.device != l.mod.weight.device for h, l in zip(have, self.layers)):
             for l in self.layers:
@@ -420,6 +447,99 @@
         F.pack_weights_f16x2_pair_multi((_lib.F16PairDesc * len(descs))(*descs))
         self._dgrad_pack_event = None
         return True
+
+    tail_ordered = _Switch("engine_tail_ordered")
+
+    tail_hook = None
+
+    _TailGroup = collections.namedtuple("_TailGroup", "index table descs layers event")
+
+    def _tail_order(self):
+        tpm = self.TPM or [None] * 3
+        groups = [[tpm[0], self.HE[0]], [self.HE[1], tpm[1], self.HE[2], tpm[2]], self.HD + [self.CTX] + self.EPM]
+        return [[l for l in g if l is not None] for g in groups]
+
+    def tail_plan(self, opt):
+        flat, maxima = opt.flat, opt.block_maxima
+        if any((l.wp_fwd if l.faces[0].kind == "f32" else l.wp6_fwd) is None for l in self.layers):
+            return None
+        key = (flat.data.data_ptr(), flat.numel, maxima.data_ptr(), tuple(flat.offsets),
+               tuple((l.mod.weight.data_ptr(), l.faces, l.taps, l.wp6_fwd.data_ptr() if l.wp6_fwd is not None else 0,
+                      l.wp6_dgrad.data_ptr() if l.wp6_dgrad is not None else 0) for l in self.layers))
+        if self._tail_cache is not None and self._tail_cache[0] == key:
+            return self._tail_cache[1]
+        self._tail_cache = (key, self._build_tail_plan(flat, maxima))
+        return self._tail_cache[1]
+
+    def _build_tail_plan(self, flat, maxima, max_ranges=40):
+        ch = F.adam_chunk()
+        order = self._tail_order()
+        group_of = {id(l.mod.weight): gi for gi, g in enumerate(order) for l in g}
+        in_flat = {id(p) for p in flat.params}
+        if any(id(l.mod.weight) not in in_flat for l in self.layers):
+            return None
+        all_ranges = tail_chunk_ranges([(off, p.numel(), group_of.get(id(p), 0)) for p, off in zip(flat.params, flat.offsets)],
+                                       flat.numel, ch, len(order))
+        plan = []
+        for gi, layers in enumerate(order):
+            ranges = all_ranges[gi]
+            descs = [l.pair_desc() for l in layers]
+            if len(ranges) > max_ranges or any(d is None for d in descs):
+                return None
+            if not all(_attach_block_maxima(d, d.A * d.B * d.R * d.S, maxima, flat.data, ch) for d in descs):
+                return None
+            if not layers and not ranges:
+                continue
+            if not layers and plan:
+                return None
+            plan.append(self._TailGroup(len(plan), F.adam_ranges(ranges), (_lib.F16PairDesc * len(descs))(*descs) if descs else None, layers,
+                                        self._events.setdefault(("tail", len(plan)), torch.cuda.Event())))
+        return plan
+
+    def run_tail(self, plan, adam):
+        dev = self.layers[0].mod.weight.device
+        main, side = F.cur_stream(dev), self.side_stream(dev)
+        adam(plan[0].table)
+        F.stream_wait(side, main)
+        if plan[0].descs is not None:
+            F.pack_weights_f16x2_pair_multi(plan[0].descs)
+        with F.on_stream(side):
+            if self.tail_hook is not None:
+                F.tape_py(self.tail_hook)
+            for g in plan[1:]:
+                adam(g.table)
+                F.pack_weights_f16x2_pair_multi(g.descs)
+                F.event_record(g.event, side)
+        self.mark_tail(plan)
+        self._dgrad_pack_event = None
+        self._pack_key = self._weights_key()
+
+    def mark_tail(self, plan):
+        self._tail_waited.clear()
+        for l in self.layers:
+            l.tail_event = None
+        for g in plan[1:]:
+            for l in g.layers:
+                l.tail_event, l.tail_group = g.event, g.index
+        self._tail_last = plan[-1].event if len(plan) > 1 else None
+
+    def _wait_tail(self, layer):
+        st = F.cur_stream()
+        key = (st.cuda_stream, layer.tail_group)
+        if key not in self._tail_waited:
+            self._tail_waited.add(key)
+            F.event_wait(st, layer.tail_event)
+
+    def join_tail(self):
+        if self._tail_last is not None:
+            F.event_wait(F.cur_stream(), self._tail_last)
+
+    def _drop_tail(self):
+        self.join_tail()
+        self._tail_last = None
+        self._tail_waited.clear()
+        for l in self.layers:
+            l.tail_event = None
 
     def unpack_all(self):
         for lane in sorted({l.lane for l in self.layers}):
diff --git a/spatiotemporalentropymodel_amd/functional.py b/spatiotemporalentropymodel_amd/functional.py
--- a/spatiotemporalentropymodel_amd/functional.py
+++ b/spatiotemporalentropymodel_amd/functional.py
@@ -1672,6 +1672,17 @@
                                         max_norm, gscale, lr, beta1, beta2, eps, step, int(bool(zero_grad)), bmax.data_ptr(), _stream()))
 
 
+def adam_ranges(ranges):
+    flat = [int(c) for r in ranges for c in r]
+    return (C.c_int * len(flat))(*flat)
+
+
+def adam_step_bmax_ranges(p, g, m, v, sumsq_acc, max_norm, gscale, lr, beta1, beta2, eps, step, bmax, table, zero_grad=False):
+    _lib.check_tail(_lib.tail().stem_adam_step_bmax_ranges(p.data_ptr(), g.data_ptr(), m.data_ptr(), v.data_ptr(), p.numel(), _ptr(sumsq_acc),
+                                                           max_norm, gscale, lr, beta1, beta2, eps, step, int(bool(zero_grad)),
+                                                           bmax.data_ptr(), table, len(table) // 2, _stream()))
+
+
 def adam_chunk():
     return int(_lib.hip().stem_adam_chunk())
 
diff --git a/spatiotemporalentropymodel_amd/optim.py b/spatiotemporalentropymodel_amd/optim.py
--- a/spatiotemporalentropymodel_amd/optim.py
+++ b/spatiotemporalentropymodel_amd/optim.py
@@ -119,9 +119,7 @@
                             float(self.max_norm) if use_clip else 0.0, float(grad_scale), d["lr"], g["betas"][0], g["betas"][1],
                             float(g["eps"]), d["step"], d["scal"])
         elif block_max:
-            if getattr(self, "block_maxima", None) is None:
-                ch = F.adam_chunk()
-                self.block_maxima = torch.empty(4 * ((self.flat.data.numel() + ch - 1) // ch), device=self.flat.data.device, dtype=torch.float32)
+            self.ensure_block_maxima()
             F.adam_step_bmax(self.flat.data, self.flat.grad, self.m, self.v, self._sumsq if use_clip else None,
                              float(self.max_norm) if use_clip else 0.0, float(grad_scale), float(g["lr"]), g["betas"][0], g["betas"][1],
                              float(g["eps"]), self.t, self.block_maxima, zero_grad=zero_grad)
@@ -135,6 +133,29 @@
                                         float(g["betas"][1]), float(g["eps"])))
         bump_weight_epoch(self.flat.params)
         return loss
+
+    def ensure_block_maxima(self):
+        if getattr(self, "block_maxima", None) is None:
+            ch = F.adam_chunk()
+            self.block_maxima = torch.empty(4 * ((self.flat.data.numel() + ch - 1) // ch), device=self.flat.data.device, dtype=torch.float32)
+        return self.block_maxima
+
+    def begin_ranges(self, grad_scale: float = 1.0):
+        assert self._dev is None, "begin_ranges: the step count lives in device memory (enable_device_state)"
+        join_wgrad_stream()
+        self.t += 1
+        self.ensure_block_maxima()
+        bump_weight_epoch(self.flat.params)
+        g, gs = self.param_groups[0], float(grad_scale)
+        use_clip = self.max_norm is not None and self.max_norm > 0
+        self._ranges_floats = (use_clip, lambda: (float(self.max_norm) if use_clip else 0.0, gs, float(g["lr"]), float(g["betas"][0]),
+                                                  float(g["betas"][1]), float(g["eps"])))
+
+    def step_ranges(self, table, zero_grad: bool = False):
+        use_clip, floats = self._ranges_floats
+        F.adam_step_bmax_ranges(self.flat.data, self.flat.grad, self.m, self.v, self._sumsq if use_clip else None, *floats(), self.t,
+                                self.block_maxima, table, zero_grad=zero_grad)
+        F.tape_bind_floats(floats)
 
     def _views(self, buf):
         return [buf[o:o + p.numel()].view(p.shape) for p, o in zip(self.flat.params, self.flat.offsets)]
diff --git a/spatiotemporalentropymodel_amd/tape.py b/spatiotemporalentropymodel_amd/tape.py
--- a/spatiotemporalentropymodel_amd/tape.py
+++ b/spatiotemporalentropymodel_amd/tape.py
@@ -30,14 +30,17 @@
         self.foreign = []
         self.problems = []
         self.float_bindings = {}
+        self.float_followers = {}
         self._bound_now = {}
         self._native = None
         self._segments = None
 
     def add_call(self, name, fn, args):
-        sig = _lib._HIP_SIG[name]
+        sig = _lib._TAPE_SIG[name]
         addr = C.cast(fn, C.c_void_p).value
-        if not _lib.hip().stem_tape_entry_recordable(addr):
+        known = (_lib.tail().stem_tail_entry_recordable(addr) if name in _lib._TAIL_SIG
+                 else _lib.hip().stem_tape_entry_recordable(addr))
+        if not known:
             self.problems.append(f"{name} is not in the library's table of recordable entry points (csrc/tape_entries.inc)")
             return
         if len(args) != len(sig):
@@ -70,17 +73,27 @@
         nf = sum(1 for k in self.entries[i][3] if k != 0)
         if len(provider()) != nf:
             raise RuntimeError(f"tape_bind_floats: {self.entries[i][1]} has {nf} float arguments, the provider returns {len(provider())}")
+        for j, other in self.float_bindings.items():
+            if other is provider:
+                self.float_followers[i] = j
+                return
         self.float_bindings[i] = provider
+
+    def _provider(self, i):
+        return self.float_bindings[self.float_followers.get(i, i)]
+
+    def _bound_entries(self):
+        return list(self.float_bindings) + list(self.float_followers)
 
     def _float_patterns(self, i):
         x = self.entries[i]
-        sig = _lib._HIP_SIG[x[1]]
+        sig = _lib._TAPE_SIG[x[1]]
         ftys = [ty for ty in sig if ty is C.c_float or ty is C.c_double]
-        return [_pattern(ty, v) for ty, v in zip(ftys, self.float_bindings[i]())]
+        return [_pattern(ty, v) for ty, v in zip(ftys, self._provider(i)())]
 
     def refresh_floats(self):
         lib, n = _lib.hip(), 0
-        for i in self.float_bindings:
+        for i in self._bound_entries():
             now = self._float_patterns(i)
             old = self._bound_now[i]
             if now != old and [struct.pack("<d", v) for v in now] != [struct.pack("<d", v) for v in old]:
@@ -100,7 +113,7 @@
         if self.foreign or second.foreign:
             ops = sorted(set(self.foreign + second.foreign))
             raise TapeRefused("LaunchTape: the step runs torch operators on device memory that a replay would drop: " + ", ".join(ops))
-        if set(self.float_bindings) != set(second.float_bindings):
+        if set(self.float_bindings) != set(second.float_bindings) or self.float_followers != second.float_followers:
             raise TapeRefused("LaunchTape: the two recordings bound different launches to float providers")
         lib = _lib.hip()
         nat = lib.stem_tape_create()
@@ -127,7 +140,7 @@
                 _, name, addr, kinds, iv, fv, _keep, isptr = x
                 self.native_index.append(lib.stem_tape_length(nat))
                 deltas = [0] * len(iv)
-                bound = ei in self.float_bindings
+                bound = ei in self.float_bindings or ei in self.float_followers
                 if bound:
                     cur = self._float_patterns(ei)
                     self._bound_now[ei] = cur
@@ -206,8 +219,8 @@
         if w is not None:
             return w
         fn = getattr(self._lib, name)
-        if (name not in _lib._HIP_SIG or name in _lib._RESTYPE or name.startswith("stem_tape_") or name.startswith("stem_tuning")
-                or name.startswith("stem_stream_flag_")):
+        if (name not in _lib._TAPE_SIG or name in _lib._RESTYPE or name.startswith("stem_tape_") or name.startswith("stem_tuning")
+                or name.startswith("stem_stream_flag_") or name.startswith("stem_tail_")):
             return fn
         tape = self._tape
 
@@ -257,6 +270,8 @@
             raise RuntimeError("a launch tape is already recording")
         self._real = _lib.hip()
         _lib._hip = _RecordingLibrary(self._real, self.tape)
+        self._real_tail = _lib.tail()
+        _lib._tail = _RecordingLibrary(self._real_tail, self.tape)
         F._TAPE = self.tape
         self._guard = _ForeignOpGuard(self.tape)
         self._guard.__enter__()
@@ -284,6 +299,7 @@
     def __exit__(self, *exc):
         self._guard.__exit__(*exc)
         _lib._hip = self._real
+        _lib._tail = self._real_tail
         F._TAPE = None
         for n, real in self._saved.items():
             setattr(torch, n, real)
@@ -322,7 +338,7 @@
         clip = tuple(bool(o.max_norm is not None and o.max_norm > 0) for o in (f.opt, f.aux_opt))
         return (tuple(y_cur.shape), tuple(y_cond.shape), tuple(y_cur.stride()), tuple(y_cond.stride()), y_cur.dtype, y_cond.dtype, y_cur.device,
                 int(num_pixels), float(grad_scale), id(reducer), F.cur_stream(y_cur.device).cuda_stream, clip, bool(f.clear_grad_in_adam),
-                bool(f.adam_block_max), bool(f.overwrite_grads))
+                bool(f.adam_block_max), bool(f.overwrite_grads), bool(f.eng.tail_ordered))
 
     def step(self, y_cur, y_cond, num_pixels, grad_scale=1.0, reducer=None):
         key = self._key(y_cur, y_cond, num_pixels, grad_scale, reducer)
@@ -409,6 +425,7 @@
     def packs_are_current(self):
         if self.tape is not None and self.replays > 1:
             self.fused.eng._pack_key = self._weights_key
+        self.fused.eng.join_tail()
 
     def finish(self):
         self.fused.finish()
diff --git a/spatiotemporalentropymodel_amd/trainer.py b/spatiotemporalentropymodel_amd/trainer.py
--- a/spatiotemporalentropymodel_amd/trainer.py
+++ b/spatiotemporalentropymodel_amd/trainer.py
@@ -117,6 +117,7 @@
         self.adam_block_max = _config.runtime().adam_block_max
         self._aux_stream = self.eng.side_stream(eb.quantiles.device) or F.make_stream(eb.quantiles.device, "side")
         self._aux_pending = False
+        self._tail_plan = None
         self._done_event = torch.cuda.Event()
 
     def step(self, y_cur, y_cond, num_pixels, grad_scale=1.0, reducer=None):
@@ -145,7 +146,17 @@
         F.sumsq(opt.flat.grad, opt._sumsq, overwrite=True)
         clean = opt._dev is None and self.clear_grad_in_adam and not overwrite
         use_bmax = opt._dev is None and eng.use_fx3 and self.adam_block_max
-        opt.step(grad_scale=grad_scale, norm_is_current=True, zero_grad=clean, block_max=use_bmax)
+        plan = None
+        if (use_bmax and eng.tail_ordered and eng.pack_pair and eng.side_stream(main.device) is self._aux_stream
+                and not torch.cuda.is_current_stream_capturing()):
+            opt.ensure_block_maxima()
+            plan = eng.tail_plan(opt)
+        self._tail_plan = plan
+        if plan is not None:
+            opt.begin_ranges(grad_scale)
+            eng.run_tail(plan, lambda table: opt.step_ranges(table, zero_grad=clean))
+        else:
+            opt.step(grad_scale=grad_scale, norm_is_current=True, zero_grad=clean, block_max=use_bmax)
         self._grad_clean = clean
         F.stream_wait(self._aux_stream, main)
         with F.on_stream(self._aux_stream):
@@ -168,6 +179,8 @@
         from .layers import bump_weight_epoch
         bump_weight_epoch(self.opt.flat.params)
         self._aux_pending = True
+        if self._tail_plan is not None:
+            self.eng.mark_tail(self._tail_plan)
 
     def finish(self):
         if self._aux_pending:
```

Measured after the change: 10290 frames/s (median of 6 runs). 1.01x the previous value.
